# otiliastr/coper

Hardware: NVIDIA B200
Metric: train_rows_per_s (higher is better)
Workload: dtype fp16x3

## Files before the change

### coper_b200/csrc/common.cuh

```cuda
#pragma once
#include <cuda_runtime.h>
#include <stdint.h>
#include "../../include/coper.h"

namespace coper {

extern thread_local int g_last_cuda_error;
extern long long g_launch_count;

inline int check_launch() {
  ++g_launch_count;
  cudaError_t e = cudaPeekAtLastError();
  if (e != cudaSuccess) {
    g_last_cuda_error = (int)e;
    cudaGetLastError();
    return COPER_ERR_CUDA;
  }
  return COPER_OK;
}
inline int check_cuda(cudaError_t e) {
  if (e != cudaSuccess) {
    g_last_cuda_error = (int)e;
    return COPER_ERR_CUDA;
  }
  return COPER_OK;
}
#define COPER_CHECK_ARG(cond) \
  do {                        \
    if (!(cond)) return COPER_ERR_INVALID_ARG; \
  } while (0)

static inline cudaStream_t as_stream(coper_stream_t s) { return reinterpret_cast<cudaStream_t>(s); }

__device__ __forceinline__ void pdl_trigger() { asm volatile("griddepcontrol.launch_dependents;" ::: "memory"); }
__device__ __forceinline__ void pdl_wait() { asm volatile("griddepcontrol.wait;" ::: "memory"); }
__device__ __forceinline__ void pdl_enter() {
  pdl_trigger();
  pdl_wait();
}
bool pdl_enabled();
template <typename... KArgs, typename... Args>
inline void launch_pdl(void (*kernel)(KArgs...), dim3 grid, dim3 block, size_t smem, cudaStream_t st, Args&&... args) {
  cudaLaunchConfig_t cfg = {};
  cfg.gridDim = grid;
  cfg.blockDim = block;
  cfg.dynamicSmemBytes = smem;
  cfg.stream = st;
  cudaLaunchAttribute attr[1];
  attr[0].id = cudaLaunchAttributeProgrammaticStreamSerialization;
  attr[0].val.programmaticStreamSerializationAllowed = pdl_enabled() ? 1 : 0;
  cfg.attrs = attr;
  cfg.numAttrs = 1;
  cudaLaunchKernelEx(&cfg, kernel, static_cast<KArgs>(args)...);
}

__host__ __device__ __forceinline__ uint32_t hash32(uint64_t seed, uint64_t idx) {
  uint64_t z = seed + (idx + 1) * 0x9E3779B97F4A7C15ull;
  z = (z ^ (z >> 30)) * 0xBF58476D1CE4E5B9ull;
  z = (z ^ (z >> 27)) * 0x94D049BB133111EBull;
  z ^= (z >> 31);
  return (uint32_t)(z >> 32);
}
__host__ __device__ __forceinline__ uint32_t keep_threshold(float keep) {
  double t = (double)keep * 4294967296.0;
  if (t >= 4294967295.0) return 0xFFFFFFFFu;
  if (t <= 0.0) return 0u;
  return (uint32_t)t;
}
__device__ __forceinline__ float drop_factor(float keep, float inv_keep, uint32_t thr, uint64_t seed, uint64_t idx) {
  if (keep >= 1.0f) return 1.0f;
  return hash32(seed, idx) < thr ? inv_keep : 0.0f;
}

__device__ __forceinline__ float bn_bwd_dx(float dout, float post_factor, float xv, float ac, float bc, float mean,
                                           float invstd, float c1, float c2, int relu) {
  float g = __fmul_rn(dout, post_factor);
  if (relu && !(fmaf(ac, xv, bc) > 0.f)) g = 0.f;
  const float xhat = __fmul_rn(__fsub_rn(xv, mean), invstd);
  return __fmul_rn(ac, fmaf(-xhat, c2, __fsub_rn(g, c1)));
}

__device__ __forceinline__ float warp_sum(float v) {
#pragma unroll
  for (int o = 16; o > 0; o >>= 1) v += __shfl_xor_sync(0xffffffffu, v, o);
  return v;
}
__device__ __forceinline__ float warp_max(float v) {
#pragma unroll
  for (int o = 16; o > 0; o >>= 1) v = fmaxf(v, __shfl_xor_sync(0xffffffffu, v, o));
  return v;
}
__device__ __forceinline__ double warp_sum_d(double v) {
#pragma unroll
  for (int o = 16; o > 0; o >>= 1) v += __shfl_xor_sync(0xffffffffu, v, o);
  return v;
}
__device__ __forceinline__ int warp_sum_i(int v) {
#pragma unroll
  for (int o = 16; o > 0; o >>= 1) v += __shfl_xor_sync(0xffffffffu, v, o);
  return v;
}

template <typename T>
__device__ __forceinline__ T block_sum(T v, T* smem32) {
  int lane = threadIdx.x & 31, w = threadIdx.x >> 5;
#pragma unroll
  for (int o = 16; o > 0; o >>= 1) v += __shfl_xor_sync(0xffffffffu, v, o);
  if (lane == 0) smem32[w] = v;
  __syncthreads();
  T r = T(0);
  if (w == 0) {
    int nw = (blockDim.x + 31) >> 5;
    r = lane < nw ? smem32[lane] : T(0);
#pragma unroll
    for (int o = 16; o > 0; o >>= 1) r += __shfl_xor_sync(0xffffffffu, r, o);
  }
  __syncthreads();
  return r;
}

constexpr int kFp16x3TargetExp = 10;
__host__ __device__ __forceinline__ int fp16x3_exponent_of(float absmax) {
  if (!(absmax > 0.f) || !(absmax < 3.0e38f)) return 0;
  int ex;
  frexpf(absmax, &ex);
  int e = kFp16x3TargetExp - (ex - 1);
  return e < -100 ? -100 : (e > 100 ? 100 : e);
}

inline int sm_count() {
  static int cached[64] = {};
  int dev = 0;
  if (cudaGetDevice(&dev) != cudaSuccess || dev < 0 || dev >= 64) return 148;
  if (!cached[dev]) {
    int n = 0;
    if (cudaDeviceGetAttribute(&n, cudaDevAttrMultiProcessorCount, dev) != cudaSuccess || n <= 0) n = 148;
    cached[dev] = n;
  }
  return cached[dev];
}

int reduce_partials_and_sum(const float* in, int S, int64_t n, float scale, int accumulate, float* out,
                            const double* dsum_in, int dsum_n, double* dsum_out, cudaStream_t st);

static inline int ceil_div(int64_t a, int64_t b) { return (int)((a + b - 1) / b); }
static inline size_t align_up(size_t x, size_t a) { return (x + a - 1) / a * a; }

}
```

### coper_b200/csrc/umma.cuh

```cuda
#pragma once
#include <cuda.h>
#include <cuda_bf16.h>
#include "common.cuh"

namespace coper {
namespace umma {

__device__ __forceinline__ uint32_t smem_u32(const void* p) { return (uint32_t)__cvta_generic_to_shared(p); }

__device__ __forceinline__ bool elect_one() {
  uint32_t pred;
  asm volatile("{\n\t.reg .pred P;\n\telect.sync _|P, 0xffffffff;\n\tselp.u32 %0, 1, 0, P;\n\t}" : "=r"(pred));
  return pred != 0;
}
__device__ __forceinline__ int warp_idx_uniform() { return __shfl_sync(0xffffffffu, (int)(threadIdx.x >> 5), 0); }

__device__ __forceinline__ void mbar_init(uint64_t* bar, uint32_t count) {
  asm volatile("mbarrier.init.shared::cta.b64 [%0], %1;" ::"r"(smem_u32(bar)), "r"(count));
}
__device__ __forceinline__ void fence_barrier_init() { asm volatile("fence.mbarrier_init.release.cluster;" ::: "memory"); }
__device__ __forceinline__ void fence_proxy_async() { asm volatile("fence.proxy.async.shared::cta;" ::: "memory"); }
__device__ __forceinline__ void mbar_expect_tx(uint64_t* bar, uint32_t bytes) {
  asm volatile("mbarrier.arrive.expect_tx.shared::cta.b64 _, [%0], %1;" ::"r"(smem_u32(bar)), "r"(bytes) : "memory");
}
__device__ __forceinline__ void mbar_arrive(uint64_t* bar) {
  asm volatile("mbarrier.arrive.shared::cta.b64 _, [%0];" ::"r"(smem_u32(bar)) : "memory");
}
__device__ __forceinline__ void mbar_wait(uint64_t* bar, uint32_t parity) {
  uint32_t addr = smem_u32(bar);
  uint32_t done = 0;
  while (!done) {
    asm volatile(
        "{\n\t.reg .pred p;\n\t"
        "mbarrier.try_wait.parity.shared::cta.b64 p, [%1], %2;\n\t"
        "selp.u32 %0, 1, 0, p;\n\t}"
        : "=r"(done)
        : "r"(addr), "r"(parity)
        : "memory");
  }
}

__device__ __forceinline__ void tma_load_2d(void* dst_smem, const CUtensorMap* tmap, uint64_t* bar, int c0, int c1) {
  asm volatile(
      "cp.async.bulk.tensor.2d.shared::cluster.global.mbarrier::complete_tx::bytes [%0], [%1, {%3, %4}], [%2];"
      ::"r"(smem_u32(dst_smem)), "l"(reinterpret_cast<uint64_t>(tmap)), "r"(smem_u32(bar)), "r"(c0), "r"(c1)
      : "memory");
}
__device__ __forceinline__ void tma_store_2d(const CUtensorMap* tmap, const void* src_smem, int c0, int c1) {
  asm volatile("cp.async.bulk.tensor.2d.global.shared::cta.bulk_group [%0, {%2, %3}], [%1];"
               ::"l"(reinterpret_cast<uint64_t>(tmap)), "r"(smem_u32(src_smem)), "r"(c0), "r"(c1)
               : "memory");
}
__device__ __forceinline__ void tma_store_commit() { asm volatile("cp.async.bulk.commit_group;" ::: "memory"); }
__device__ __forceinline__ void tma_store_wait_read() { asm volatile("cp.async.bulk.wait_group.read 0;" ::: "memory"); }
__device__ __forceinline__ void tma_store_wait_all() { asm volatile("cp.async.bulk.wait_group 0;" ::: "memory"); }
__device__ __forceinline__ void mbar_wait_guarded(uint64_t* bar, uint32_t parity) {
  uint32_t addr = smem_u32(bar);
  uint32_t done = 0;
  long long t0 = 0;
  for (uint32_t spins = 0; !done; ++spins) {
    asm volatile(
        "{\n\t.reg .pred p;\n\t"
        "mbarrier.try_wait.parity.shared::cta.b64 p, [%1], %2;\n\t"
        "selp.u32 %0, 1, 0, p;\n\t}"
        : "=r"(done)
        : "r"(addr), "r"(parity)
        : "memory");
    if (!done && (spins & 1023u) == 1023u) {
      long long now = clock64();
      if (t0 == 0) t0 = now;
      else if (now - t0 > 4000000000ll) __trap();
    }
  }
}
__device__ __forceinline__ void tma_prefetch_l2_2d(const CUtensorMap* tmap, int c0, int c1) {
  asm volatile("cp.async.bulk.prefetch.tensor.2d.L2.global.tile [%0, {%1, %2}];"
               ::"l"(reinterpret_cast<uint64_t>(tmap)), "r"(c0), "r"(c1)
               : "memory");
}
__device__ __forceinline__ void tma_prefetch_desc(const CUtensorMap* tmap) {
  asm volatile("prefetch.tensormap [%0];" ::"l"(reinterpret_cast<uint64_t>(tmap)) : "memory");
}

__device__ __forceinline__ void tmem_alloc(uint32_t* smem_dst, uint32_t ncols) {
  asm volatile("tcgen05.alloc.cta_group::1.sync.aligned.shared::cta.b32 [%0], %1;" ::"r"(smem_u32(smem_dst)), "r"(ncols)
               : "memory");
}
__device__ __forceinline__ void tmem_relinquish() {
  asm volatile("tcgen05.relinquish_alloc_permit.cta_group::1.sync.aligned;" ::: "memory");
}
__device__ __forceinline__ void tmem_dealloc(uint32_t taddr, uint32_t ncols) {
  asm volatile("tcgen05.dealloc.cta_group::1.sync.aligned.b32 %0, %1;" ::"r"(taddr), "r"(ncols) : "memory");
}
__device__ __forceinline__ void tc_fence_before() { asm volatile("tcgen05.fence::before_thread_sync;" ::: "memory"); }
__device__ __forceinline__ void tc_fence_after() { asm volatile("tcgen05.fence::after_thread_sync;" ::: "memory"); }

__device__ __forceinline__ void mma_bf16(uint32_t tmem_d, uint64_t desc_a, uint64_t desc_b, uint32_t idesc, uint32_t acc) {
  asm volatile(
      "{\n\t.reg .pred p;\n\tsetp.ne.b32 p, %4, 0;\n\t"
      "tcgen05.mma.cta_group::1.kind::f16 [%0], %1, %2, %3, p;\n\t}"
      ::"r"(tmem_d), "l"(desc_a), "l"(desc_b), "r"(idesc), "r"(acc)
      : "memory");
}
__device__ __forceinline__ void mma_tf32(uint32_t tmem_d, uint64_t desc_a, uint64_t desc_b, uint32_t idesc, uint32_t acc) {
  asm volatile(
      "{\n\t.reg .pred p;\n\tsetp.ne.b32 p, %4, 0;\n\t"
      "tcgen05.mma.cta_group::1.kind::tf32 [%0], %1, %2, %3, p;\n\t}"
      ::"r"(tmem_d), "l"(desc_a), "l"(desc_b), "r"(idesc), "r"(acc)
      : "memory");
}
__device__ __forceinline__ void mma_commit(uint64_t* bar) {
  asm volatile("tcgen05.commit.cta_group::1.mbarrier::arrive::one.shared::cluster.b64 [%0];" ::"r"(smem_u32(bar))
               : "memory");
}

__device__ __forceinline__ void tmem_ld32(uint32_t taddr, uint32_t (&r)[32]) {
  asm volatile(
      "tcgen05.ld.sync.aligned.32x32b.x32.b32 "
      "{%0, %1, %2, %3, %4, %5, %6, %7, %8, %9, %10, %11, %12, %13, %14, %15, "
      "%16, %17, %18, %19, %20, %21, %22, %23, %24, %25, %26, %27, %28, %29, %30, %31}, [%32];"
      : "=r"(r[0]), "=r"(r[1]), "=r"(r[2]), "=r"(r[3]), "=r"(r[4]), "=r"(r[5]), "=r"(r[6]), "=r"(r[7]), "=r"(r[8]),
        "=r"(r[9]), "=r"(r[10]), "=r"(r[11]), "=r"(r[12]), "=r"(r[13]), "=r"(r[14]), "=r"(r[15]), "=r"(r[16]),
        "=r"(r[17]), "=r"(r[18]), "=r"(r[19]), "=r"(r[20]), "=r"(r[21]), "=r"(r[22]), "=r"(r[23]), "=r"(r[24]),
        "=r"(r[25]), "=r"(r[26]), "=r"(r[27]), "=r"(r[28]), "=r"(r[29]), "=r"(r[30]), "=r"(r[31])
      : "r"(taddr)
      : "memory");
}
__device__ __forceinline__ void tmem_ld16(uint32_t taddr, uint32_t (&r)[16]) {
  asm volatile(
      "tcgen05.ld.sync.aligned.32x32b.x16.b32 "
      "{%0, %1, %2, %3, %4, %5, %6, %7, %8, %9, %10, %11, %12, %13, %14, %15}, [%16];"
      : "=r"(r[0]), "=r"(r[1]), "=r"(r[2]), "=r"(r[3]), "=r"(r[4]), "=r"(r[5]), "=r"(r[6]), "=r"(r[7]), "=r"(r[8]),
        "=r"(r[9]), "=r"(r[10]), "=r"(r[11]), "=r"(r[12]), "=r"(r[13]), "=r"(r[14]), "=r"(r[15])
      : "r"(taddr)
      : "memory");
}
__device__ __forceinline__ void tmem_ld_wait() { asm volatile("tcgen05.wait::ld.sync.aligned;" ::: "memory"); }

enum : uint32_t { LAYOUT_SW128 = 2, LAYOUT_SW128_BASE32B = 1 };
__device__ __forceinline__ uint64_t make_desc(uint32_t smem_addr, uint32_t lbo_bytes, uint32_t sbo_bytes,
                                              uint32_t layout_type = LAYOUT_SW128) {
  uint64_t d = 0;
  d |= (uint64_t)((smem_addr & 0x3FFFFu) >> 4);
  d |= (uint64_t)((lbo_bytes >> 4) & 0x3FFFu) << 16;
  d |= (uint64_t)((sbo_bytes >> 4) & 0x3FFFu) << 32;
  d |= (uint64_t)1 << 46;
  d |= (uint64_t)layout_type << 61;
  return d;
}
__device__ __forceinline__ uint64_t make_desc_kmajor(uint32_t smem_addr) { return make_desc(smem_addr, 16, 1024); }

enum : uint32_t { FMT_F16 = 0, FMT_BF16 = 1, FMT_TF32 = 2 };
__host__ __device__ constexpr uint32_t make_idesc(uint32_t fmt, uint32_t M, uint32_t N, uint32_t a_mn, uint32_t b_mn) {
  return (1u << 4) | (fmt << 7) | (fmt << 10) | (a_mn << 15) | (b_mn << 16) | ((N >> 3) << 17) | ((M >> 4) << 24);
}

typedef CUresult (*EncodeTiledFn)(CUtensorMap*, CUtensorMapDataType, cuuint32_t, void*, const cuuint64_t*,
                                  const cuuint64_t*, const cuuint32_t*, const cuuint32_t*, CUtensorMapInterleave,
                                  CUtensorMapSwizzle, CUtensorMapL2promotion, CUtensorMapFloatOOBfill);
EncodeTiledFn get_encode_fn();

int make_tmap_2d(CUtensorMap* out, const void* base, int elem_bytes, bool is_bf16, uint64_t rows, uint64_t cols,
                 uint64_t pitch_elems, uint32_t box_cols, uint32_t box_rows, bool atom32 = false);

}
}
```

### coper_b200/csrc/umma_cpg.cu

```cuda
#include <cuda_fp16.h>
#include "umma_gemm.cuh"

namespace coper {
using namespace umma;

size_t tc_prepared_bytes(int64_t rows, int cols, int prec);
int tc_prepare(const float* src, int64_t rows, int cols, int64_t ld_src, int prec, void* dst, cudaStream_t st);
int64_t tc_prepared_ld(int cols, int prec);
TcOperand tc_operand(const void* prep, int64_t rows, int cols, int prec);
void* tc_fp16x3_trailer(const void* prep, int64_t rows, int cols);
int tc_gemm_store(int prec, bool a_mn, bool b_mn, const TcOperand& A, const TcOperand& B, const GemmProblem& p,
                  bool split, const StoreEpi& epi, cudaStream_t st);

struct CpgFwdEpi : EpiBase {
  static constexpr bool kAccumulate = true;
  const float* c;
  int dc;
  float* out;
  long long ld, split_stride;
  __device__ __forceinline__ float group_scale(const GemmProblem& p, const TileCoord& t, int row) const {
    return row < p.M ? __ldg(c + (long long)row * dc + t.group) : 0.f;
  }
  __device__ __forceinline__ void chunk(const GemmProblem& p, const TileCoord& t, int row, int col,
                                        const uint32_t (&r)[32], int) const {
    if (row >= p.M) return;
    float* o = out + t.split * split_stride + (long long)row * ld + col;
    if (col + 31 < p.N && ((reinterpret_cast<uintptr_t>(o) & 15) == 0)) {
#pragma unroll
      for (int j = 0; j < 32; j += 4)
        *reinterpret_cast<float4*>(o + j) = make_float4(__uint_as_float(r[j]), __uint_as_float(r[j + 1]),
                                                        __uint_as_float(r[j + 2]), __uint_as_float(r[j + 3]));
    } else {
#pragma unroll
      for (int j = 0; j < 32; ++j)
        if (col + j < p.N) o[j] = __uint_as_float(r[j]);
    }
  }
};

template <int PREC>
using CpgFwdCfg = GemmCfg<PREC, 256, (PREC == PREC_BF16 ? 4 : 2), 8, false, true,
                          (PREC == PREC_BF16 ? 0 : PREC == PREC_FP16X3 ? 2 : 4)>;

struct CpgFwdPlan {
  GemmProblem p;
  size_t off_f, off_P, off_slabs, total;
};
static CpgFwdPlan cpg_fwd_plan(int B, int dc, int F, int d, int prec) {
  CpgFwdPlan L;
  GemmProblem p{};
  p.M = B; p.N = d; p.K = F; p.groups = dc; p.groups_inner = 1;
  p.a_group_mn = 0; p.a_group_k = 0; p.b_group_mn = 0; p.b_group_k = F;
  if (prec == COPER_PREC_BF16) plan_gemm<CpgFwdCfg<PREC_BF16>>(p, true);
  else if (prec == COPER_PREC_FP16X3) plan_gemm<CpgFwdCfg<PREC_FP16X3>>(p, true);
  else plan_gemm<CpgFwdCfg<PREC_TF32X3>>(p, true);
  L.p = p;
  size_t o = 0;
  L.off_f = o; o = align_up(o + tc_prepared_bytes(B, F, prec), 256);
  L.off_P = o; o = align_up(o + tc_prepared_bytes((int64_t)dc * F, d, prec), 256);
  L.off_slabs = o; o = align_up(o + (size_t)p.splits * B * d * sizeof(float), 256);
  L.total = o;
  return L;
}

struct CpgBwdTEpi : EpiBase {
  static constexpr bool kAccumulate = true;
  const float* c;
  const float* f;
  int dc;
  float* df;
  float* dc_part;
  float freg[32];
  float fsum;
  __device__ __forceinline__ void tile_begin(const GemmProblem& p, const TileCoord&, int row, int col0) {
    fsum = 0.f;
    if (row < p.M && col0 < p.N) {
      const float4* src = reinterpret_cast<const float4*>(f + (long long)row * p.N + col0);
#pragma unroll
      for (int j = 0; j < 8; ++j) {
        float4 v = __ldg(src + j);
        freg[4 * j] = v.x; freg[4 * j + 1] = v.y; freg[4 * j + 2] = v.z; freg[4 * j + 3] = v.w;
      }
    } else {
#pragma unroll
      for (int j = 0; j < 32; ++j) freg[j] = 0.f;
    }
  }
  __device__ __forceinline__ float group_scale(const GemmProblem& p, const TileCoord& t, int row) const {
    return row < p.M ? __ldg(c + (long long)row * dc + t.group) : 0.f;
  }
  __device__ __forceinline__ void group_vals(const GemmProblem&, const TileCoord&, int, int, const uint32_t (&v)[16],
                                             int half_idx) {
#pragma unroll
    for (int j = 0; j < 16; ++j) fsum = fmaf(freg[(half_idx & 1) * 16 + j], __uint_as_float(v[j]), fsum);
  }
  __device__ __forceinline__ void group_done(const GemmProblem& p, const TileCoord& t, int row, int col_group,
                                             int col_groups) {
    if (row < p.M)
      dc_part[((long long)(t.n_blk * col_groups + col_group) * p.M + row) * dc + t.group] = fsum;
    fsum = 0.f;
  }
  __device__ __forceinline__ void chunk(const GemmProblem& p, const TileCoord&, int row, int col,
                                        const uint32_t (&r)[32], int) const {
    if (row >= p.M) return;
    float4* o = reinterpret_cast<float4*>(df + (long long)row * p.N + col);
#pragma unroll
    for (int j = 0; j < 8; ++j)
      o[j] = make_float4(__uint_as_float(r[4 * j]), __uint_as_float(r[4 * j + 1]), __uint_as_float(r[4 * j + 2]),
                         __uint_as_float(r[4 * j + 3]));
  }
};
constexpr int kBwdTEpiWarps = 16;
constexpr int kBwdTBlockN = 128;
template <int PREC>
using CpgBwdTCfg = GemmCfg<PREC, kBwdTBlockN, (PREC == PREC_BF16 ? 4 : 3), kBwdTEpiWarps, false, false, 0>;

__global__ void absmax_scaled_kernel(const float* __restrict__ dy, const float* __restrict__ c, int B, int d, int dc,
                                     uint32_t* __restrict__ trailer) {
  pdl_enter();
  const int lane = threadIdx.x & 31;
  for (int b = blockIdx.x * (blockDim.x >> 5) + (threadIdx.x >> 5); b < B; b += gridDim.x * (blockDim.x >> 5)) {
    float my = 0.f, mc = 0.f;
    for (int j = lane; j < d; j += 32) my = fmaxf(my, fabsf(__ldg(dy + (int64_t)b * d + j)));
    for (int g = lane; g < dc; g += 32) mc = fmaxf(mc, fabsf(__ldg(c + (int64_t)b * dc + g)));
#pragma unroll
    for (int o = 16; o > 0; o >>= 1) {
      my = fmaxf(my, __shfl_xor_sync(0xffffffffu, my, o));
      mc = fmaxf(mc, __shfl_xor_sync(0xffffffffu, mc, o));
    }
    const float m = my * mc;
    if (lane == 0 && m > 0.f) atomicMax(trailer + 1, __float_as_uint(m));
  }
}
__global__ void prepare_scaled_kernel(const float* __restrict__ dy, const float* __restrict__ c, int B, int d, int dc,
                                      int64_t ldp, int prec, void* __restrict__ dst, uint32_t* __restrict__ trailer) {
  pdl_enter();
  int64_t n = (int64_t)dc * B * ldp;
  int64_t stride = (int64_t)gridDim.x * blockDim.x;
  float sc = 1.0f;
  if (prec == COPER_PREC_FP16X3) {
    const int ex = fp16x3_exponent_of(__uint_as_float(trailer[1]));
    if (blockIdx.x == 0 && threadIdx.x == 0) reinterpret_cast<int*>(trailer)[0] = ex;
    sc = exp2f((float)ex);
  }
  for (int64_t e = (int64_t)blockIdx.x * blockDim.x + threadIdx.x; e < n; e += stride) {
    int64_t r = e / ldp;
    int j = (int)(e - r * ldp);
    int g = (int)(r / B), b = (int)(r - (int64_t)g * B);
    float x = j < d ? __ldg(dy + (int64_t)b * d + j) * __ldg(c + (int64_t)b * dc + g) : 0.f;
    if (prec == COPER_PREC_BF16) {
      static_cast<__nv_bfloat16*>(dst)[e] = __float2bfloat16_rn(x);
    } else if (prec == COPER_PREC_FP16X3) {
      const float xs = x * sc;
      const __half h = __float2half_rn(xs);
      static_cast<__half*>(dst)[e] = h;
      static_cast<__half*>(dst)[n + e] = __float2half_rn(xs - __half2float(h));
    } else {
      uint32_t h;
      asm("cvt.rna.tf32.f32 %0, %1;" : "=r"(h) : "f"(x));
      float hf = __uint_as_float(h);
      static_cast<float*>(dst)[e] = hf;
      static_cast<float*>(dst)[n + e] = x - hf;
    }
  }
}

__global__ void __launch_bounds__(256) cpg_bwd_prepare_fp16x3_kernel(const float* __restrict__ dy,
                                                                     const float* __restrict__ c, int B, int d, int dc,
                                                                     int64_t ldp, __half* __restrict__ dyp,
                                                                     __half* __restrict__ dycp,
                                                                     uint32_t* __restrict__ tr_dy,
                                                                     uint32_t* __restrict__ tr_dyc) {
  pdl_enter();
  __shared__ float wmax[2][8];
  const int lane = threadIdx.x & 31, warp = threadIdx.x >> 5;
  float m_dy = 0.f, m_dyc = 0.f;
  for (int b = blockIdx.x * 8 + warp; b < B; b += gridDim.x * 8) {
    float my = 0.f, mc = 0.f;
    for (int j = lane; j < d; j += 32) my = fmaxf(my, fabsf(__ldg(dy + (int64_t)b * d + j)));
    for (int g = lane; g < dc; g += 32) mc = fmaxf(mc, fabsf(__ldg(c + (int64_t)b * dc + g)));
    my = warp_max(my);
    mc = warp_max(mc);
    m_dy = fmaxf(m_dy, my);
    m_dyc = fmaxf(m_dyc, my * mc);
  }
  if (lane == 0) { wmax[0][warp] = m_dy; wmax[1][warp] = m_dyc; }
  __syncthreads();
  if (threadIdx.x == 0) {
#pragma unroll
    for (int w = 1; w < 8; ++w) { m_dy = fmaxf(m_dy, wmax[0][w]); m_dyc = fmaxf(m_dyc, wmax[1][w]); }
    if (m_dy > 0.f) atomicMax(tr_dy + 1, __float_as_uint(m_dy));
    if (m_dyc > 0.f) atomicMax(tr_dy + 4, __float_as_uint(m_dyc));
    __threadfence();
    atomicAdd(tr_dy + 3, 1u);
    const long long t0 = clock64();
    while (*reinterpret_cast<volatile uint32_t*>(tr_dy + 3) < gridDim.x) {
      if (clock64() - t0 > 4000000000ll) __trap();
    }
    __threadfence();
  }
  __syncthreads();
  const uint32_t bits_dy = *reinterpret_cast<volatile uint32_t*>(tr_dy + 1);
  const uint32_t bits_dyc = *reinterpret_cast<volatile uint32_t*>(tr_dy + 4);
  const int e_dy = fp16x3_exponent_of(__uint_as_float(bits_dy)), e_dyc = fp16x3_exponent_of(__uint_as_float(bits_dyc));
  if (blockIdx.x == 0 && threadIdx.x == 0) {
    reinterpret_cast<int*>(tr_dy)[0] = e_dy;
    tr_dy[2] = bits_dy;
    reinterpret_cast<int*>(tr_dyc)[0] = e_dyc;
    tr_dyc[1] = bits_dyc;
  }
  const float sc_dy = exp2f((float)e_dy), sc_dyc = exp2f((float)e_dyc);
  const int gpr = (int)(ldp / 8);
  const int64_t per = (int64_t)B * gpr, units = per * (1 + dc);
  __half* const dy_lo = dyp + (int64_t)B * ldp;
  __half* const dyc_lo = dycp + (int64_t)dc * B * ldp;
  for (int64_t u = (int64_t)blockIdx.x * 256 + threadIdx.x; u < units; u += (int64_t)gridDim.x * 256) {
    const int p = (int)(u / per);
    const int64_t v = u - (int64_t)p * per;
    const int b = (int)(v / gpr), c0 = (int)(v - (int64_t)b * gpr) * 8;
    const float cs = p == 0 ? 1.0f : __ldg(c + (int64_t)b * dc + (p - 1));
    const float sc = p == 0 ? sc_dy : sc_dyc;
    __half2 h[4], l[4];
#pragma unroll
    for (int k = 0; k < 4; ++k) {
      const int j = c0 + 2 * k;
      float x0 = j < d ? __ldg(dy + (int64_t)b * d + j) : 0.f, x1 = j + 1 < d ? __ldg(dy + (int64_t)b * d + j + 1) : 0.f;
      if (p != 0) { x0 = j < d ? x0 * cs : 0.f; x1 = j + 1 < d ? x1 * cs : 0.f; }
      const float a0 = x0 * sc, a1 = x1 * sc;
      h[k] = __floats2half2_rn(a0, a1);
      const float2 hf = __half22float2(h[k]);
      l[k] = __floats2half2_rn(a0 - hf.x, a1 - hf.y);
    }
    __half* hi = p == 0 ? dyp + v * 8 : dycp + ((int64_t)(p - 1) * per + v) * 8;
    __half* lo = p == 0 ? dy_lo + v * 8 : dyc_lo + ((int64_t)(p - 1) * per + v) * 8;
    *reinterpret_cast<uint4*>(hi) = *reinterpret_cast<uint4*>(h);
    *reinterpret_cast<uint4*>(lo) = *reinterpret_cast<uint4*>(l);
  }
}

struct CpgBwdPlan {
  size_t off_f, off_P, off_dy, off_dyc, off_dcpart, total;
  int dc_slabs;
};
static CpgBwdPlan cpg_bwd_plan(int B, int dc, int F, int d, int prec) {
  CpgBwdPlan L;
  size_t o = 0;
  L.off_f = o; o = align_up(o + tc_prepared_bytes(B, F, prec), 256);
  L.off_P = o; o = align_up(o + tc_prepared_bytes((int64_t)dc * F, d, prec), 256);
  L.off_dy = o; o = align_up(o + tc_prepared_bytes(B, d, prec), 256);
  L.off_dyc = o; o = align_up(o + tc_prepared_bytes((int64_t)dc * B, d, prec), 256);
  L.dc_slabs = ((F + kBwdTBlockN - 1) / kBwdTBlockN) * (kBwdTEpiWarps / 4);
  L.off_dcpart = o; o = align_up(o + (size_t)L.dc_slabs * B * dc * sizeof(float), 256);
  L.total = o;
  return L;
}

size_t umma_cpg_fwd_workspace_bytes(int B, int dc, int F, int d, int prec) { return cpg_fwd_plan(B, dc, F, d, prec).total; }
size_t umma_cpg_bwd_workspace_bytes(int B, int dc, int F, int d, int prec) {
  size_t a = cpg_bwd_plan(B, dc, F, d, prec).total, b = cpg_fwd_plan(B, dc, F, d, prec).total;
  return a > b ? a : b;
}

int umma_cpg_fwd_partials(const float* c, const float* f, const float* P, const void* P_prepared, int B, int dc, int F,
                          int d, void* ws, size_t ws_bytes, int prec, cudaStream_t st, float** slabs, int* n_slabs) {
  if (F % 32 != 0 || d > 256) return COPER_ERR_UNSUPPORTED;
  CpgFwdPlan L = cpg_fwd_plan(B, dc, F, d, prec);
  if (!ws || ws_bytes < L.total) return COPER_ERR_WORKSPACE;
  if (reinterpret_cast<uintptr_t>(ws) & 255) return COPER_ERR_INVALID_ARG;
  char* w = static_cast<char*>(ws);
  void* fp = w + L.off_f;
  const void* Pp = P_prepared ? P_prepared : w + L.off_P;
  float* out = reinterpret_cast<float*>(w + L.off_slabs);
  int rc;
  if ((rc = tc_prepare(f, B, F, F, prec, fp, st))) return rc;
  if (!P_prepared && (rc = tc_prepare(P, (int64_t)dc * F, d, d, prec, w + L.off_P, st))) return rc;
  CpgFwdEpi epi;
  epi.c = c; epi.dc = dc; epi.out = out; epi.ld = d; epi.split_stride = (long long)B * d;
  TcOperand A = tc_operand(fp, B, F, prec), Bo = tc_operand(Pp, (int64_t)dc * F, d, prec);
  if (prec == COPER_PREC_BF16) rc = launch_gemm<CpgFwdCfg<PREC_BF16>, CpgFwdEpi>(A, Bo, L.p, epi, st);
  else if (prec == COPER_PREC_FP16X3) rc = launch_gemm<CpgFwdCfg<PREC_FP16X3>, CpgFwdEpi>(A, Bo, L.p, epi, st);
  else rc = launch_gemm<CpgFwdCfg<PREC_TF32X3>, CpgFwdEpi>(A, Bo, L.p, epi, st);
  *slabs = out;
  *n_slabs = L.p.splits;
  return rc;
}

int umma_cpg_bwd(const float* c, const float* f, const float* P, const void* P_prepared, const float* dy, int B, int dc,
                 int F, int d, float* dP, float* df, float* dc_out, void* ws, size_t ws_bytes, int prec,
                 int flags, cudaStream_t st) {
  if (F % 32 != 0 || d > 256) return COPER_ERR_UNSUPPORTED;
  const bool inputs = !(flags & COPER_CPG_BWD_WEIGHT_GRADS_ONLY), weights = !(flags & COPER_CPG_BWD_INPUT_GRADS_ONLY);
  CpgBwdPlan L = cpg_bwd_plan(B, dc, F, d, prec);
  if (!ws || ws_bytes < L.total) return COPER_ERR_WORKSPACE;
  if (reinterpret_cast<uintptr_t>(ws) & 255) return COPER_ERR_INVALID_ARG;
  char* w = static_cast<char*>(ws);
  void* fp = w + L.off_f;
  const void* Pp = P_prepared ? P_prepared : w + L.off_P;
  void* dyp = w + L.off_dy;
  void* dycp = w + L.off_dyc;
  float* dc_part = reinterpret_cast<float*>(w + L.off_dcpart);
  int rc = COPER_OK;
  if (inputs) {
    if (!(flags & COPER_CPG_BWD_REUSE_FWD)) {
      if ((rc = tc_prepare(f, B, F, F, prec, fp, st))) return rc;
      if (!P_prepared && (rc = tc_prepare(P, (int64_t)dc * F, d, d, prec, w + L.off_P, st))) return rc;
    }
    int64_t ldp = tc_prepared_ld(d, prec);
    int64_t n = (int64_t)dc * B * ldp;
    if (prec == COPER_PREC_FP16X3 && n <= ((int64_t)8 << 20)) {
      uint32_t* tr_dy = static_cast<uint32_t*>(tc_fp16x3_trailer(dyp, B, d));
      uint32_t* tr_dyc = static_cast<uint32_t*>(tc_fp16x3_trailer(dycp, (int64_t)dc * B, d));
      if ((rc = check_cuda(cudaMemsetAsync(tr_dy, 0, 32, st)))) return rc;
      const int64_t want = ((int64_t)(1 + dc) * B * (ldp / 8) + 256 * 4 - 1) / (256 * 4);
      int g = (int)(want < (int64_t)sm_count() * 2 ? want : (int64_t)sm_count() * 2);
      if (g < 1) g = 1;
      launch_pdl(cpg_bwd_prepare_fp16x3_kernel, g, 256, 0, st, dy, c, B, d, dc, ldp, static_cast<__half*>(dyp),
                 static_cast<__half*>(dycp), tr_dy, tr_dyc);
      if ((rc = check_launch())) return rc;
    } else {
      if ((rc = tc_prepare(dy, B, d, d, prec, dyp, st))) return rc;
      int grid = (int)((n + 255) / 256 < sm_count() * 8 ? (n + 255) / 256 : sm_count() * 8);
      uint32_t* trailer = nullptr;
      if (prec == COPER_PREC_FP16X3) {
        trailer = static_cast<uint32_t*>(tc_fp16x3_trailer(dycp, (int64_t)dc * B, d));
        if ((rc = check_cuda(cudaMemsetAsync(trailer, 0, 8, st)))) return rc;
        launch_pdl(absmax_scaled_kernel, (B + 7) / 8, 256, 0, st, dy, c, B, d, dc, trailer);
        if ((rc = check_launch())) return rc;
      }
      launch_pdl(prepare_scaled_kernel, grid, 256, 0, st, dy, c, B, d, dc, ldp, prec, dycp, trailer);
      if ((rc = check_launch())) return rc;
    }
    GemmProblem p{};
    p.M = B; p.N = F; p.K = d; p.groups = dc; p.groups_inner = 1;
    p.a_group_mn = 0; p.a_group_k = 0; p.b_group_mn = F; p.b_group_k = 0;
    CpgBwdTEpi epi;
    epi.c = c; epi.f = f; epi.dc = dc; epi.df = df; epi.dc_part = dc_part; epi.fsum = 0.f;
    TcOperand A = tc_operand(dyp, B, d, prec), Bo = tc_operand(Pp, (int64_t)dc * F, d, prec);
    if (prec == COPER_PREC_BF16) {
      plan_gemm<CpgBwdTCfg<PREC_BF16>>(p, false);
      rc = launch_gemm<CpgBwdTCfg<PREC_BF16>, CpgBwdTEpi>(A, Bo, p, epi, st);
    } else if (prec == COPER_PREC_FP16X3) {
      plan_gemm<CpgBwdTCfg<PREC_FP16X3>>(p, false);
      rc = launch_gemm<CpgBwdTCfg<PREC_FP16X3>, CpgBwdTEpi>(A, Bo, p, epi, st);
    } else {
      plan_gemm<CpgBwdTCfg<PREC_TF32X3>>(p, false);
      rc = launch_gemm<CpgBwdTCfg<PREC_TF32X3>, CpgBwdTEpi>(A, Bo, p, epi, st);
    }
    if (rc) return rc;
    if ((rc = coper_reduce_partials(dc_part, L.dc_slabs, (int64_t)B * dc, 1.0f, 0, dc_out, (coper_stream_t)st)))
      return rc;
  }
  if (weights) {
    GemmProblem p{};
    p.M = F; p.N = d; p.K = B; p.groups = dc; p.groups_inner = 0;
    p.a_group_mn = 0; p.a_group_k = 0; p.b_group_mn = 0; p.b_group_k = B;
    StoreEpi epi = make_store_epi(dP, d, (long long)F * d, 0);
    rc = tc_gemm_store(prec, true, true, tc_operand(fp, B, F, prec), tc_operand(dycp, (int64_t)dc * B, d, prec), p,
                       false, epi, st);
  }
  return rc;
}

}
```

### coper_b200/csrc/umma_gemm.cu

```cuda
#include "umma_gemm.cuh"

namespace coper {
using namespace umma;

size_t tc_prepared_bytes(int64_t rows, int cols, int prec);
int tc_prepare(const float* src, int64_t rows, int cols, int64_t ld_src, int prec, void* dst, cudaStream_t st);
int64_t tc_prepared_ld(int cols, int prec);
void* tc_fp16x3_trailer(const void* prep, int64_t rows, int cols);

template <int PREC, bool A_MN, bool B_MN>
using StoreCfg = GemmCfg<PREC, 256, (PREC == PREC_BF16 ? 4 : 2), (PREC == PREC_BF16 ? 4 : 8), A_MN, B_MN,
                         (PREC == PREC_BF16 ? 0 : PREC == PREC_FP16X3 ? 2 : 4)>;

template <int PREC>
static int dispatch_layout(bool a_mn, bool b_mn, const TcOperand& A, const TcOperand& B, GemmProblem p, bool split,
                           const StoreEpi& epi, cudaStream_t st) {
  if (!a_mn && !b_mn) { plan_gemm<StoreCfg<PREC, false, false>>(p, split); return launch_gemm<StoreCfg<PREC, false, false>>(A, B, p, epi, st); }
  if (!a_mn && b_mn)  { plan_gemm<StoreCfg<PREC, false, true>>(p, split);  return launch_gemm<StoreCfg<PREC, false, true>>(A, B, p, epi, st); }
  if (a_mn && !b_mn)  { plan_gemm<StoreCfg<PREC, true, false>>(p, split);  return launch_gemm<StoreCfg<PREC, true, false>>(A, B, p, epi, st); }
  plan_gemm<StoreCfg<PREC, true, true>>(p, split);
  return launch_gemm<StoreCfg<PREC, true, true>>(A, B, p, epi, st);
}

using ResBCfg = GemmCfg<PREC_BF16, 128, 4, 8, false, true, 0, 8>;
int tc_gemm_store_resident_b(const TcOperand& A, const TcOperand& B, GemmProblem p, const StoreEpi& epi, cudaStream_t st) {
  plan_gemm<ResBCfg>(p, false);
  return launch_gemm<ResBCfg>(A, B, p, epi, st);
}
bool tc_resident_b_ok(int prec, bool a_mn, bool b_mn, const GemmProblem& p) {
  return prec == COPER_PREC_BF16 && !a_mn && b_mn && p.groups == 1 && p.K <= ResBCfg::RES_KB * ResBCfg::BLOCK_K &&
         p.M >= 16 * BLOCK_M;
}

int tc_gemm_store(int prec, bool a_mn, bool b_mn, const TcOperand& A, const TcOperand& B, const GemmProblem& p,
                  bool split, const StoreEpi& epi, cudaStream_t st) {
  if (prec == COPER_PREC_BF16) return dispatch_layout<PREC_BF16>(a_mn, b_mn, A, B, p, split, epi, st);
  if (prec == COPER_PREC_TF32X3) return dispatch_layout<PREC_TF32X3>(a_mn, b_mn, A, B, p, split, epi, st);
  if (prec == COPER_PREC_FP16X3) return dispatch_layout<PREC_FP16X3>(a_mn, b_mn, A, B, p, split, epi, st);
  return COPER_ERR_UNSUPPORTED;
}
int tc_plan_splits(int prec, GemmProblem p, bool split) {
  if (prec == COPER_PREC_BF16) plan_gemm<StoreCfg<PREC_BF16, false, false>>(p, split);
  else if (prec == COPER_PREC_FP16X3) plan_gemm<StoreCfg<PREC_FP16X3, false, false>>(p, split);
  else plan_gemm<StoreCfg<PREC_TF32X3, false, false>>(p, split);
  return p.splits;
}

TcOperand tc_operand(const void* prep, int64_t rows, int cols, int prec) {
  TcOperand o;
  int64_t ldp = tc_prepared_ld(cols, prec);
  o.main = prep;
  o.lo = prec == COPER_PREC_TF32X3 ? static_cast<const void*>(static_cast<const float*>(prep) + rows * ldp)
         : prec == COPER_PREC_FP16X3 ? static_cast<const void*>(static_cast<const uint16_t*>(prep) + rows * ldp)
                                     : nullptr;
  o.exp = prec == COPER_PREC_FP16X3 ? static_cast<const int*>(tc_fp16x3_trailer(prep, rows, cols)) : nullptr;
  o.rows = (uint64_t)rows;
  o.cols = (uint64_t)cols;
  o.pitch = (uint64_t)ldp;
  return o;
}
}

using namespace coper;

extern "C" {

size_t coper_tc_gemm_workspace_bytes(int M, int N, int K, int prec) {
  size_t a = tc_prepared_bytes(M > K ? M : K, M > K ? K : M, prec) + tc_prepared_bytes(K, M, prec);
  size_t b = tc_prepared_bytes(N > K ? N : K, N > K ? K : N, prec) + tc_prepared_bytes(K, N, prec);
  return a + b + 1024;
}

int coper_tc_gemm(int transA, int transB, int M, int N, int K, const float* A, int lda, const float* B, int ldb,
                  float* C, int ldc, int prec, void* workspace, size_t workspace_bytes, coper_stream_t stream) {
  COPER_CHECK_ARG(A && B && C && workspace && M > 0 && N > 0 && K > 0 && ldc >= N);
  if (prec != COPER_PREC_BF16 && prec != COPER_PREC_TF32X3 && prec != COPER_PREC_FP16X3) return COPER_ERR_UNSUPPORTED;
  if (workspace_bytes < coper_tc_gemm_workspace_bytes(M, N, K, prec)) return COPER_ERR_WORKSPACE;
  cudaStream_t st = as_stream(stream);
  char* p = reinterpret_cast<char*>((reinterpret_cast<uintptr_t>(workspace) + 255) & ~uintptr_t(255));
  int64_t a_rows = transA ? K : M, a_cols = transA ? M : K;
  int64_t b_rows = transB ? N : K, b_cols = transB ? K : N;
  void* Ap = p;
  void* Bp = p + tc_prepared_bytes(a_rows, (int)a_cols, prec);
  int rc;
  if ((rc = tc_prepare(A, a_rows, (int)a_cols, lda, prec, Ap, st))) return rc;
  if ((rc = tc_prepare(B, b_rows, (int)b_cols, ldb, prec, Bp, st))) return rc;
  GemmProblem g{};
  g.M = M; g.N = N; g.K = K; g.groups = 1; g.groups_inner = 0;
  StoreEpi epi = make_store_epi(C, ldc, 0, 0);
  return tc_gemm_store(prec, transA != 0, transB == 0, tc_operand(Ap, a_rows, (int)a_cols, prec),
                       tc_operand(Bp, b_rows, (int)b_cols, prec), g, false, epi, st);
}

}
```

### coper_b200/csrc/umma_gemm.cuh

```cuda
#pragma once
#include "umma.cuh"

namespace coper {
namespace umma {

constexpr int PREC_BF16 = COPER_PREC_BF16, PREC_TF32X3 = COPER_PREC_TF32X3, PREC_FP16X3 = COPER_PREC_FP16X3;
constexpr int BLOCK_M = 128;
constexpr int NUM_NON_EPI_THREADS = 128;

template <int PREC_, int BLOCK_N_, int STAGES_, int EPI_WARPS_, bool A_MN_, bool B_MN_, int PROMOTE_KB_ = 0,
          int RES_KB_ = 0>
struct GemmCfg {
  static constexpr int PROMOTE_KB = PROMOTE_KB_;
  static constexpr int RES_KB = RES_KB_;
  static constexpr int PREC = PREC_, BLOCK_N = BLOCK_N_, STAGES = STAGES_, EPI_WARPS = EPI_WARPS_;
  static constexpr bool A_MN = A_MN_, B_MN = B_MN_;
  static constexpr int ELEM = (PREC == PREC_TF32X3) ? 4 : 2;
  static constexpr int CHUNK = 128 / ELEM;
  static constexpr int BLOCK_K = CHUNK;
  static constexpr int UMMA_K = 32 / ELEM;
  static constexpr int TERMS = (PREC == PREC_BF16) ? 1 : 2;
  static constexpr bool SCALED = (PREC == PREC_FP16X3);
  static constexpr int A_BYTES = BLOCK_M * 128;
  static constexpr int B_BYTES = BLOCK_N * 128;
  static constexpr int STAGE_BYTES = RES_KB_ > 0 ? TERMS * A_BYTES : TERMS * (A_BYTES + B_BYTES);
  static constexpr int RES_BYTES = RES_KB_ * TERMS * B_BYTES;
  static constexpr int TMEM_COLS = (2 * BLOCK_N <= 32) ? 32 : (2 * BLOCK_N <= 64) ? 64 : (2 * BLOCK_N <= 128) ? 128
                                   : (2 * BLOCK_N <= 256) ? 256 : 512;
  static constexpr int THREADS = NUM_NON_EPI_THREADS + EPI_WARPS * 32;
  static constexpr size_t SMEM_BYTES = (size_t)STAGES * STAGE_BYTES + RES_BYTES + 1024  + 256 ;

  static constexpr uint32_t FMT = (PREC == PREC_BF16) ? FMT_BF16 : (PREC == PREC_FP16X3) ? FMT_F16 : FMT_TF32;
  static constexpr bool MN_ATOM32 = (PREC == PREC_TF32X3);
  static constexpr uint32_t MN_LAYOUT = MN_ATOM32 ? LAYOUT_SW128_BASE32B : LAYOUT_SW128;
  static constexpr uint32_t MN_SBO = MN_ATOM32 ? 512 : 1024;
  static constexpr uint32_t IDESC = make_idesc(FMT, BLOCK_M, BLOCK_N, A_MN ? 1u : 0u, B_MN ? 1u : 0u);
  static_assert(BLOCK_N % 16 == 0 && BLOCK_N >= 16 && BLOCK_N <= 256, "UMMA N");
  static_assert(2 * BLOCK_N <= 512, "TMEM double buffer");
  static_assert(!A_MN || (BLOCK_M % CHUNK == 0), "MN-major A chunking");
  static_assert(!B_MN || (BLOCK_N % CHUNK == 0), "MN-major B chunking");
};

template <class Cfg>
struct SmemLayout {
  uint8_t* base;
  uint64_t* full;
  uint64_t* empty;
  uint64_t* tfull;
  uint64_t* tempty;
  uint64_t* bfull;
  uint32_t* tmem_ptr;
  uint8_t* res;
  __device__ __forceinline__ explicit SmemLayout(uint8_t* raw) {
    base = reinterpret_cast<uint8_t*>((reinterpret_cast<uintptr_t>(raw) + 1023) & ~uintptr_t(1023));
    res = base + (size_t)Cfg::STAGES * Cfg::STAGE_BYTES;
    uint64_t* bars = reinterpret_cast<uint64_t*>(res + Cfg::RES_BYTES);
    full = bars;
    empty = bars + Cfg::STAGES;
    tfull = bars + 2 * Cfg::STAGES;
    tempty = tfull + 2;
    bfull = tempty + 2;
    tmem_ptr = reinterpret_cast<uint32_t*>(bfull + 1);
  }
  __device__ __forceinline__ uint8_t* res_plane(int kb, int term) const {
    return res + ((size_t)kb * Cfg::TERMS + term) * Cfg::B_BYTES;
  }
  __device__ __forceinline__ uint8_t* a_plane(int stage, int term) const {
    return base + (size_t)stage * Cfg::STAGE_BYTES + term * Cfg::A_BYTES;
  }
  __device__ __forceinline__ uint8_t* b_plane(int stage, int term) const {
    return base + (size_t)stage * Cfg::STAGE_BYTES + Cfg::TERMS * Cfg::A_BYTES + term * Cfg::B_BYTES;
  }
};

template <class Cfg>
__device__ __forceinline__ uint32_t cta_setup(const SmemLayout<Cfg>& sm) {
  int warp = threadIdx.x >> 5;
  if (warp == 1 && (threadIdx.x & 31) == 0) {
    for (int i = 0; i < Cfg::STAGES; ++i) { mbar_init(&sm.full[i], 1); mbar_init(&sm.empty[i], 1); }
    for (int i = 0; i < 2; ++i) { mbar_init(&sm.tfull[i], 1); mbar_init(&sm.tempty[i], Cfg::EPI_WARPS); }
    mbar_init(sm.bfull, 1);
    fence_barrier_init();
  } else if (warp == 2) {
    tmem_alloc(sm.tmem_ptr, Cfg::TMEM_COLS);
    tmem_relinquish();
  }
  tc_fence_before();
  __syncthreads();
  tc_fence_after();
  return *sm.tmem_ptr;
}
template <class Cfg>
__device__ __forceinline__ void cta_teardown(uint32_t tmem_base) {
  tc_fence_before();
  __syncthreads();
  if ((threadIdx.x >> 5) == 2) {
    tc_fence_after();
    tmem_dealloc(tmem_base, Cfg::TMEM_COLS);
  }
}

template <class Cfg>
__device__ __forceinline__ void produce_stage(const SmemLayout<Cfg>& sm, int stage, const CUtensorMap* tA,
                                              const CUtensorMap* tAlo, const CUtensorMap* tB, const CUtensorMap* tBlo,
                                              int a_mn0, int b_mn0, int a_k0, int b_k0, bool leader) {
  uint64_t* bar = &sm.full[stage];
  if (leader) mbar_expect_tx(bar, Cfg::STAGE_BYTES);
#pragma unroll
  for (int t = 0; t < Cfg::TERMS; ++t) {
    const CUtensorMap* ma = t ? tAlo : tA;
    const CUtensorMap* mb = t ? tBlo : tB;
    if (!Cfg::A_MN) {
      if (leader) tma_load_2d(sm.a_plane(stage, t), ma, bar, a_k0, a_mn0);
    } else {
#pragma unroll
      for (int c = 0; c < BLOCK_M / Cfg::CHUNK; ++c)
        if (leader) tma_load_2d(sm.a_plane(stage, t) + c * (Cfg::BLOCK_K * 128), ma, bar, a_mn0 + c * Cfg::CHUNK, a_k0);
    }
    if (Cfg::RES_KB > 0) {
    } else if (!Cfg::B_MN) {
      if (leader) tma_load_2d(sm.b_plane(stage, t), mb, bar, b_k0, b_mn0);
    } else {
#pragma unroll
      for (int c = 0; c < Cfg::BLOCK_N / Cfg::CHUNK; ++c)
        if (leader) tma_load_2d(sm.b_plane(stage, t) + c * (Cfg::BLOCK_K * 128), mb, bar, b_mn0 + c * Cfg::CHUNK, b_k0);
    }
  }
}

template <class Cfg>
__device__ __forceinline__ void issue_stage_rt(const SmemLayout<Cfg>& sm, int stage, uint32_t tmem_d, int kvalid,
                                               bool first, uint32_t idesc, int kb_res, bool leader) {
  const int nk = (kvalid + Cfg::UMMA_K - 1) / Cfg::UMMA_K;
  uint64_t da[2], db[2];
#pragma unroll
  for (int t = 0; t < Cfg::TERMS; ++t) {
    const uint32_t a_addr = smem_u32(sm.a_plane(stage, t));
    const uint32_t b_addr = smem_u32(Cfg::RES_KB > 0 ? sm.res_plane(kb_res, t) : sm.b_plane(stage, t));
    da[t] = Cfg::A_MN ? make_desc(a_addr, Cfg::BLOCK_K * 128, Cfg::MN_SBO, Cfg::MN_LAYOUT) : make_desc_kmajor(a_addr);
    db[t] = Cfg::B_MN ? make_desc(b_addr, Cfg::BLOCK_K * 128, Cfg::MN_SBO, Cfg::MN_LAYOUT) : make_desc_kmajor(b_addr);
  }
  constexpr uint64_t a_step = (Cfg::A_MN ? Cfg::UMMA_K * 128 : 32) >> 4, b_step = (Cfg::B_MN ? Cfg::UMMA_K * 128 : 32) >> 4;
  constexpr int NK_MAX = Cfg::BLOCK_K / Cfg::UMMA_K;
  if (leader) {
#pragma unroll
    for (int k = 0; k < NK_MAX; ++k) {
      if (k < nk) {
        const uint32_t acc = (first && k == 0) ? 0u : 1u;
        if (Cfg::PREC == PREC_BF16) {
          mma_bf16(tmem_d, da[0] + k * a_step, db[0] + k * b_step, idesc, acc);
        } else if (Cfg::PREC == PREC_FP16X3) {
          mma_bf16(tmem_d, da[1] + k * a_step, db[0] + k * b_step, idesc, acc);
          mma_bf16(tmem_d, da[0] + k * a_step, db[1] + k * b_step, idesc, 1u);
          mma_bf16(tmem_d, da[0] + k * a_step, db[0] + k * b_step, idesc, 1u);
        } else {
          mma_tf32(tmem_d, da[1] + k * a_step, db[0] + k * b_step, idesc, acc);
          mma_tf32(tmem_d, da[0] + k * a_step, db[1] + k * b_step, idesc, 1u);
          mma_tf32(tmem_d, da[0] + k * a_step, db[0] + k * b_step, idesc, 1u);
        }
      }
    }
  }
  __syncwarp();
}

struct PipeState {
  int stage = 0;
  uint32_t phase = 0;
  template <int STAGES>
  __device__ __forceinline__ void advance() {
    if (++stage == STAGES) { stage = 0; phase ^= 1; }
  }
};

}
}

namespace coper {
namespace umma {

struct GemmProblem {
  int M, N, K;
  int m_tiles, n_tiles;
  int splits, kb_per_split;
  int groups;
  int groups_inner;
  int a_group_mn, a_group_k;
  int b_group_mn, b_group_k;
  const int* exp_a;
  const int* exp_b;
  float post_scale;
  int n_fastest;
};
struct TileCoord {
  int group, split, m_blk, n_blk, kb0, kb1;
};

struct EpiBase {
  static constexpr bool kAccumulate = false;
  __device__ __forceinline__ void tile_begin(const GemmProblem&, const TileCoord&, int, int) {}
  __device__ __forceinline__ void tile_prefetch(const GemmProblem&, const TileCoord&, int, int) {}
  __device__ __forceinline__ float group_scale(const GemmProblem&, const TileCoord&, int) const { return 1.0f; }
  __device__ __forceinline__ void group_vals(const GemmProblem&, const TileCoord&, int, int, const uint32_t (&)[16],
                                             int) {}
  __device__ __forceinline__ void group_done(const GemmProblem&, const TileCoord&, int, int, int) {}
  __device__ __forceinline__ void tile_done(const GemmProblem&, const TileCoord&, int, int, int) {}
  __device__ __forceinline__ void finish(int, int) {}
};

__device__ __forceinline__ long long gemm_supers(const GemmProblem& p) {
  return (long long)p.m_tiles * p.n_tiles * p.splits * (p.groups_inner ? 1 : p.groups);
}
__device__ __forceinline__ TileCoord gemm_decode(const GemmProblem& p, long long s, int g_inner, int block_k) {
  TileCoord t;
  if (p.n_fastest) {
    t.n_blk = (int)(s % p.n_tiles); s /= p.n_tiles;
    t.m_blk = (int)(s % p.m_tiles); s /= p.m_tiles;
  } else {
    t.m_blk = (int)(s % p.m_tiles); s /= p.m_tiles;
    t.n_blk = (int)(s % p.n_tiles); s /= p.n_tiles;
  }
  t.split = (int)(s % p.splits);  s /= p.splits;
  t.group = p.groups_inner ? g_inner : (int)s;
  int kb_total = (p.K + block_k - 1) / block_k;
  t.kb0 = t.split * p.kb_per_split;
  t.kb1 = min(kb_total, t.kb0 + p.kb_per_split);
  return t;
}

template <class Cfg, class Epi>
__global__ void __launch_bounds__(Cfg::THREADS, 1)
umma_gemm_kernel(const __grid_constant__ CUtensorMap tA, const __grid_constant__ CUtensorMap tAlo,
                 const __grid_constant__ CUtensorMap tB, const __grid_constant__ CUtensorMap tBlo,
                 const GemmProblem p, Epi epi) {
  coper::pdl_trigger();
  extern __shared__ uint8_t smem_raw[];
  SmemLayout<Cfg> sm(smem_raw);
  uint32_t tmem_base = cta_setup<Cfg>(sm);
  coper::pdl_wait();
  const int warp = warp_idx_uniform(), lane = threadIdx.x & 31;
  const long long supers = gemm_supers(p);
  const int g_loop = p.groups_inner ? p.groups : 1;

  if (warp == 0) {
    const bool leader = elect_one();
    if (leader) {
      tma_prefetch_desc(&tA);
      tma_prefetch_desc(&tB);
    }
    PipeState ps;
    int res_nblk = -1;
    for (long long s = blockIdx.x; s < supers; s += gridDim.x) {
      for (int g = 0; g < g_loop; ++g) {
        TileCoord t = gemm_decode(p, s, g, Cfg::BLOCK_K);
        int a_mn0 = t.m_blk * BLOCK_M + t.group * p.a_group_mn;
        int b_mn0 = t.n_blk * Cfg::BLOCK_N + t.group * p.b_group_mn;
        if (Cfg::RES_KB > 0 && t.n_blk != res_nblk) {
          PipeState q = ps;
          for (int i = 0; i < Cfg::STAGES; ++i) {
            mbar_wait(&sm.empty[q.stage], q.phase ^ 1);
            q.template advance<Cfg::STAGES>();
          }
          const int kbn = t.kb1 - t.kb0;
          if (leader) mbar_expect_tx(sm.bfull, (uint32_t)(kbn * Cfg::TERMS * Cfg::B_BYTES));
          for (int kb = t.kb0; kb < t.kb1; ++kb)
#pragma unroll
            for (int tm = 0; tm < Cfg::TERMS; ++tm) {
              if (!Cfg::B_MN) {
                if (leader)
                  tma_load_2d(sm.res_plane(kb - t.kb0, tm), tm ? &tBlo : &tB, sm.bfull, kb * Cfg::BLOCK_K, b_mn0);
              } else {
#pragma unroll
                for (int c = 0; c < Cfg::BLOCK_N / Cfg::CHUNK; ++c)
                  if (leader)
                    tma_load_2d(sm.res_plane(kb - t.kb0, tm) + c * (Cfg::BLOCK_K * 128), tm ? &tBlo : &tB, sm.bfull,
                                b_mn0 + c * Cfg::CHUNK, kb * Cfg::BLOCK_K);
              }
            }
          res_nblk = t.n_blk;
        }
        for (int kb = t.kb0; kb < t.kb1; ++kb) {
          mbar_wait(&sm.empty[ps.stage], ps.phase ^ 1);
          produce_stage<Cfg>(sm, ps.stage, &tA, &tAlo, &tB, &tBlo, a_mn0, b_mn0,
                             kb * Cfg::BLOCK_K + t.group * p.a_group_k, kb * Cfg::BLOCK_K + t.group * p.b_group_k, leader);
          ps.template advance<Cfg::STAGES>();
        }
      }
    }
    __syncwarp();
  } else if (warp == 1) {
    const bool leader = elect_one();
    PipeState ps;
    int as = 0;
    uint32_t aphase = 0;
    int res_nblk = -1;
    uint32_t bphase = 0;
    for (long long s = blockIdx.x; s < supers; s += gridDim.x) {
      for (int g = 0; g < g_loop; ++g) {
        TileCoord t = gemm_decode(p, s, g, Cfg::BLOCK_K);
        if (Cfg::RES_KB > 0 && t.n_blk != res_nblk) {
          mbar_wait(sm.bfull, bphase);
          bphase ^= 1;
          res_nblk = t.n_blk;
        }
        int n_rem = p.N - t.n_blk * Cfg::BLOCK_N;
        int n_eff = min(Cfg::BLOCK_N, (n_rem + 15) & ~15);
        uint32_t idesc = make_idesc(Cfg::FMT, BLOCK_M, (uint32_t)n_eff, Cfg::A_MN ? 1u : 0u, Cfg::B_MN ? 1u : 0u);
        const int chain = Cfg::PROMOTE_KB > 0 ? Cfg::PROMOTE_KB : (t.kb1 - t.kb0);
        for (int kc = t.kb0; kc < t.kb1; kc += chain) {
          int kce = min(t.kb1, kc + chain);
          mbar_wait(&sm.tempty[as], aphase ^ 1);
          tc_fence_after();
          for (int kb = kc; kb < kce; ++kb) {
            mbar_wait(&sm.full[ps.stage], ps.phase);
            tc_fence_after();
            int kvalid = min(Cfg::BLOCK_K, p.K - kb * Cfg::BLOCK_K);
            issue_stage_rt<Cfg>(sm, ps.stage, tmem_base + as * Cfg::BLOCK_N, kvalid, kb == kc, idesc, kb - t.kb0, leader);
            if (leader) mma_commit(&sm.empty[ps.stage]);
            ps.template advance<Cfg::STAGES>();
          }
          if (leader) mma_commit(&sm.tfull[as]);
          __syncwarp();
          as ^= 1;
          if (as == 0) aphase ^= 1;
        }
      }
    }
  } else if (warp >= 4) {
    const int quarter = warp & 3;
    const int group_c = (warp - 4) >> 2;
    constexpr int GROUPS = Cfg::EPI_WARPS / 4;
    constexpr int COLS = Cfg::BLOCK_N / GROUPS;
    constexpr int NCH = COLS / 32;
    static_assert(COLS % 32 == 0, "epilogue column split");
    int as = 0;
    uint32_t aphase = 0;
    const uint32_t lane_base = (uint32_t)(quarter * 32) << 16;
    float acc_scale = 1.0f;
    if (Cfg::SCALED) {
      const int e = (p.exp_a ? __ldg(p.exp_a) : 0) + (p.exp_b ? __ldg(p.exp_b) : 0);
      acc_scale = exp2f((float)-e) * (p.post_scale != 0.f ? p.post_scale : 1.0f);
    }
    for (long long s = blockIdx.x; s < supers; s += gridDim.x) {
      TileCoord t = gemm_decode(p, s, 0, Cfg::BLOCK_K);
      const int row = t.m_blk * BLOCK_M + quarter * 32 + lane;
      const int col0 = t.n_blk * Cfg::BLOCK_N + group_c * COLS;
      epi.tile_begin(p, t, row, col0);
      if (s + gridDim.x < supers) {
        const TileCoord t2 = gemm_decode(p, s + gridDim.x, 0, Cfg::BLOCK_K);
        epi.tile_prefetch(p, t2, t2.m_blk * BLOCK_M + quarter * 32 + lane, t2.n_blk * Cfg::BLOCK_N + group_c * COLS);
      }
      if constexpr (Cfg::PROMOTE_KB == 0 && !Epi::kAccumulate) {
        mbar_wait(&sm.tfull[as], aphase);
        tc_fence_after();
#pragma unroll
        for (int i = 0; i < NCH; ++i) {
          const int col = col0 + i * 32;
          if (col < p.N) {
            uint32_t r[32];
            tmem_ld32(tmem_base + as * Cfg::BLOCK_N + group_c * COLS + i * 32 + lane_base, r);
            tmem_ld_wait();
            if (Cfg::SCALED) {
#pragma unroll
              for (int j = 0; j < 32; ++j) r[j] = __float_as_uint(__uint_as_float(r[j]) * acc_scale);
            }
            epi.chunk(p, t, row, col, r, i);
          }
        }
        tc_fence_before();
        __syncwarp();
        if (lane == 0) mbar_arrive(&sm.tempty[as]);
        as ^= 1;
        if (as == 0) aphase ^= 1;
      } else {
        float accr[NCH][32];
#pragma unroll
        for (int i = 0; i < NCH; ++i)
#pragma unroll
          for (int j = 0; j < 32; ++j) accr[i][j] = 0.f;
        for (int g = 0; g < g_loop; ++g) {
          t = gemm_decode(p, s, g, Cfg::BLOCK_K);
          const float scale = epi.group_scale(p, t, row);
          const int chain = Cfg::PROMOTE_KB > 0 ? Cfg::PROMOTE_KB : (t.kb1 - t.kb0);
          for (int kc = t.kb0; kc < t.kb1; kc += chain) {
            mbar_wait(&sm.tfull[as], aphase);
            tc_fence_after();
#pragma unroll
            for (int i = 0; i < NCH; ++i) {
              if (col0 + i * 32 < p.N) {
#pragma unroll
                for (int h = 0; h < 2; ++h) {
                  uint32_t r[16];
                  tmem_ld16(tmem_base + as * Cfg::BLOCK_N + group_c * COLS + i * 32 + h * 16 + lane_base, r);
                  tmem_ld_wait();
                  if (Cfg::SCALED) {
#pragma unroll
                    for (int j = 0; j < 16; ++j) r[j] = __float_as_uint(__uint_as_float(r[j]) * acc_scale);
                  }
                  epi.group_vals(p, t, row, col0 + i * 32 + h * 16, r, i * 2 + h);
#pragma unroll
                  for (int j = 0; j < 16; ++j) accr[i][h * 16 + j] = fmaf(scale, __uint_as_float(r[j]), accr[i][h * 16 + j]);
                }
              }
            }
            tc_fence_before();
            __syncwarp();
            if (lane == 0) mbar_arrive(&sm.tempty[as]);
            as ^= 1;
            if (as == 0) aphase ^= 1;
          }
          epi.group_done(p, t, row, group_c, GROUPS);
        }
#pragma unroll
        for (int i = 0; i < NCH; ++i) {
          const int col = col0 + i * 32;
          if (col < p.N) {
            uint32_t r[32];
#pragma unroll
            for (int j = 0; j < 32; ++j) r[j] = __float_as_uint(accr[i][j]);
            epi.chunk(p, t, row, col, r, i);
          }
        }
      }
      epi.tile_done(p, t, row, group_c, GROUPS);
    }
    epi.finish(threadIdx.x - NUM_NON_EPI_THREADS, Cfg::EPI_WARPS * 32);
  }
  cta_teardown<Cfg>(tmem_base);
}

struct TcOperand {
  const void* main;
  const void* lo;
  const int* exp;
  uint64_t rows, cols;
  uint64_t pitch;
};

template <class Cfg>
int make_gemm_tmaps(const TcOperand& A, const TcOperand& B, CUtensorMap* tA, CUtensorMap* tAlo, CUtensorMap* tB,
                    CUtensorMap* tBlo) {
  constexpr bool bf16 = Cfg::ELEM == 2;
  int rc;
  uint32_t a_box_rows = Cfg::A_MN ? Cfg::BLOCK_K : BLOCK_M;
  uint32_t b_box_rows = Cfg::B_MN ? Cfg::BLOCK_K : Cfg::BLOCK_N;
  const bool a32 = Cfg::A_MN && Cfg::MN_ATOM32, b32 = Cfg::B_MN && Cfg::MN_ATOM32;
  if ((rc = make_tmap_2d(tA, A.main, Cfg::ELEM, bf16, A.rows, A.cols, A.pitch, Cfg::CHUNK, a_box_rows, a32))) return rc;
  if ((rc = make_tmap_2d(tB, B.main, Cfg::ELEM, bf16, B.rows, B.cols, B.pitch, Cfg::CHUNK, b_box_rows, b32))) return rc;
  *tAlo = *tA;
  *tBlo = *tB;
  if (Cfg::TERMS == 2) {
    if (!A.lo || !B.lo) return COPER_ERR_INVALID_ARG;
    if ((rc = make_tmap_2d(tAlo, A.lo, Cfg::ELEM, bf16, A.rows, A.cols, A.pitch, Cfg::CHUNK, a_box_rows, a32))) return rc;
    if ((rc = make_tmap_2d(tBlo, B.lo, Cfg::ELEM, bf16, B.rows, B.cols, B.pitch, Cfg::CHUNK, b_box_rows, b32))) return rc;
  }
  return COPER_OK;
}

template <class Cfg, class Epi>
int launch_gemm(const TcOperand& A, const TcOperand& B, const GemmProblem& p, const Epi& epi, cudaStream_t st,
                int grid_override = 0) {
  if (p.groups_inner && !Epi::kAccumulate) return COPER_ERR_INVALID_ARG;
  if (Cfg::RES_KB > 0 && (p.splits != 1 || p.groups != 1 || (p.K + Cfg::BLOCK_K - 1) / Cfg::BLOCK_K > Cfg::RES_KB))
    return COPER_ERR_UNSUPPORTED;
  CUtensorMap tA, tAlo, tB, tBlo;
  int rc = make_gemm_tmaps<Cfg>(A, B, &tA, &tAlo, &tB, &tBlo);
  if (rc) return rc;
  int dev = 0;
  if ((rc = check_cuda(cudaGetDevice(&dev)))) return rc;
  static bool attr_done[64] = {};
  if (dev < 0 || dev >= 64) return COPER_ERR_UNSUPPORTED;
  if (!attr_done[dev]) {
    rc = check_cuda(cudaFuncSetAttribute(umma_gemm_kernel<Cfg, Epi>, cudaFuncAttributeMaxDynamicSharedMemorySize,
                                         (int)Cfg::SMEM_BYTES));
    if (rc) return rc;
    attr_done[dev] = true;
  }
  GemmProblem pp = p;
  if (Cfg::SCALED) {
    if (!pp.exp_a) pp.exp_a = A.exp;
    if (!pp.exp_b) pp.exp_b = B.exp;
  }
  const int sms = sm_count();
  long long supers = (long long)p.m_tiles * p.n_tiles * p.splits * (p.groups_inner ? 1 : p.groups);
  int grid = (int)(supers < sms ? supers : sms);
  if (grid_override > 0 && grid_override < grid) grid = grid_override;
  if (grid < 1) return COPER_ERR_INVALID_ARG;
  launch_pdl(umma_gemm_kernel<Cfg, Epi>, grid, Cfg::THREADS, Cfg::SMEM_BYTES, st, tA, tAlo, tB, tBlo, pp, epi);
  return check_launch();
}

template <class Cfg>
inline void plan_gemm(GemmProblem& p, bool allow_split, int target_ctas = 0) {
  if (target_ctas <= 0) target_ctas = sm_count();
  p.m_tiles = (p.M + BLOCK_M - 1) / BLOCK_M;
  p.n_tiles = (p.N + Cfg::BLOCK_N - 1) / Cfg::BLOCK_N;
  int kb_total = (p.K + Cfg::BLOCK_K - 1) / Cfg::BLOCK_K;
  long long base = (long long)p.m_tiles * p.n_tiles * (p.groups_inner ? 1 : p.groups);
  int splits = 1;
  if (allow_split && base < target_ctas) {
    splits = (int)((target_ctas + base - 1) / base);
    if (splits > kb_total) splits = kb_total;
  }
  p.kb_per_split = (kb_total + splits - 1) / splits;
  p.splits = (kb_total + p.kb_per_split - 1) / p.kb_per_split;
}

__device__ __forceinline__ void staged_store_f32(float4* st, const float (&v)[32], float* out0, long long ld,
                                                 int rows_valid, int cols_valid) {
  const int lane = threadIdx.x & 31;
#pragma unroll
  for (int g = 0; g < 8; ++g)
    st[lane * 8 + (g ^ (lane & 7))] = make_float4(v[4 * g], v[4 * g + 1], v[4 * g + 2], v[4 * g + 3]);
  __syncwarp();
  const int g = lane & 7;
#pragma unroll
  for (int k = 0; k < 8; ++k) {
    const int rr = 4 * k + (lane >> 3);
    const float4 x = st[rr * 8 + (g ^ (rr & 7))];
    if (rr < rows_valid && 4 * g < cols_valid) *reinterpret_cast<float4*>(out0 + (long long)rr * ld + 4 * g) = x;
  }
  __syncwarp();
}
constexpr int kStageWarps = 8;
__device__ __forceinline__ float4* stage_tile() {
  __shared__ float4 stage_s[kStageWarps][256];
  return stage_s[((threadIdx.x >> 5) - 4) & (kStageWarps - 1)];
}

struct StoreEpi : EpiBase {
  float* out;
  long long ld, group_stride, split_stride;
  const float* row_scale;
  int row_scale_ld;
  const float* col_bias;
  int extra_col;
  float* extra_out;
  double* sumsq_part;
  double ss_acc;
  __device__ __forceinline__ void chunk(const GemmProblem& p, const TileCoord& t, int row, int col,
                                        const uint32_t (&r)[32], int) {
    const int lane = threadIdx.x & 31;
    const int n_out = extra_col >= 0 ? min(p.N, extra_col) : p.N;
    if (sumsq_part && row < p.M) {
      float ss = 0.f;
#pragma unroll
      for (int j = 0; j < 32; ++j) {
        const float v = __uint_as_float(r[j]);
        ss = (col + j < n_out) ? fmaf(v, v, ss) : ss;
      }
      ss_acc += (double)ss;
    }
    float* base = out + t.group * group_stride + t.split * split_stride;
    float* o0 = base + (long long)(row - lane) * ld + col;
    const bool vec = !col_bias && !row_scale && extra_col < 0 && ((ld & 3) == 0) && ((n_out & 3) == 0) &&
                     ((reinterpret_cast<uintptr_t>(o0) & 15) == 0);
    if (vec) {
      float v[32];
#pragma unroll
      for (int j = 0; j < 32; ++j) v[j] = __uint_as_float(r[j]);
      staged_store_f32(stage_tile(), v, o0, ld, p.M - (row - lane), n_out - col);
      return;
    }
    if (row >= p.M) return;
    float sc = row_scale ? __ldg(row_scale + (long long)row * row_scale_ld + t.group) : 1.0f;
    float* o = base + (long long)row * ld + col;
    {
#pragma unroll
      for (int j = 0; j < 32; ++j) {
        int cj = col + j;
        if (cj < n_out) o[j] = __uint_as_float(r[j]) * sc + (col_bias ? __ldg(col_bias + cj) : 0.f);
        else if (cj == extra_col && cj < p.N) extra_out[row] = __uint_as_float(r[j]) * sc;
      }
    }
  }
  __device__ __forceinline__ void finish(int epi_thread, int epi_threads) {
    if (!sumsq_part) return;
    const double t = warp_sum_d(ss_acc);
    if ((epi_thread & 31) == 0) sumsq_part[(long long)blockIdx.x * (epi_threads >> 5) + (epi_thread >> 5)] = t;
  }
};

inline StoreEpi make_store_epi(float* out, long long ld, long long group_stride, long long split_stride) {
  StoreEpi e;
  e.out = out; e.ld = ld; e.group_stride = group_stride; e.split_stride = split_stride;
  e.row_scale = nullptr; e.row_scale_ld = 0; e.col_bias = nullptr; e.extra_col = -1; e.extra_out = nullptr;
  e.sumsq_part = nullptr; e.ss_acc = 0.0;
  return e;
}

}
}
```

Measured before the change: 999,900.

## Use 2-SM paired UMMA (cta_group::2) clusters for forward and store GEMMs

```diff
diff --git a/coper_b200/csrc/common.cuh b/coper_b200/csrc/common.cuh
--- a/coper_b200/csrc/common.cuh
+++ b/coper_b200/csrc/common.cuh
@@ -40,18 +40,25 @@
 }
 bool pdl_enabled();
 template <typename... KArgs, typename... Args>
-inline void launch_pdl(void (*kernel)(KArgs...), dim3 grid, dim3 block, size_t smem, cudaStream_t st, Args&&... args) {
+inline void launch_pdl_cluster(void (*kernel)(KArgs...), int cluster_x, dim3 grid, dim3 block, size_t smem,
+                               cudaStream_t st, Args&&... args) {
   cudaLaunchConfig_t cfg = {};
   cfg.gridDim = grid;
   cfg.blockDim = block;
   cfg.dynamicSmemBytes = smem;
   cfg.stream = st;
-  cudaLaunchAttribute attr[1];
+  cudaLaunchAttribute attr[2];
   attr[0].id = cudaLaunchAttributeProgrammaticStreamSerialization;
   attr[0].val.programmaticStreamSerializationAllowed = pdl_enabled() ? 1 : 0;
+  attr[1].id = cudaLaunchAttributeClusterDimension;
+  attr[1].val.clusterDim.x = (unsigned)cluster_x; attr[1].val.clusterDim.y = 1; attr[1].val.clusterDim.z = 1;
   cfg.attrs = attr;
-  cfg.numAttrs = 1;
+  cfg.numAttrs = cluster_x > 1 ? 2 : 1;
   cudaLaunchKernelEx(&cfg, kernel, static_cast<KArgs>(args)...);
+}
+template <typename... KArgs, typename... Args>
+inline void launch_pdl(void (*kernel)(KArgs...), dim3 grid, dim3 block, size_t smem, cudaStream_t st, Args&&... args) {
+  launch_pdl_cluster(kernel, 1, grid, block, smem, st, static_cast<Args&&>(args)...);
 }
 
 __host__ __device__ __forceinline__ uint32_t hash32(uint64_t seed, uint64_t idx) {
diff --git a/coper_b200/csrc/umma.cuh b/coper_b200/csrc/umma.cuh
--- a/coper_b200/csrc/umma.cuh
+++ b/coper_b200/csrc/umma.cuh
@@ -82,36 +82,110 @@
   asm volatile("prefetch.tensormap [%0];" ::"l"(reinterpret_cast<uint64_t>(tmap)) : "memory");
 }
 
+template <bool PAIR = false>
 __device__ __forceinline__ void tmem_alloc(uint32_t* smem_dst, uint32_t ncols) {
-  asm volatile("tcgen05.alloc.cta_group::1.sync.aligned.shared::cta.b32 [%0], %1;" ::"r"(smem_u32(smem_dst)), "r"(ncols)
-               : "memory");
-}
+  if constexpr (PAIR)
+    asm volatile("tcgen05.alloc.cta_group::2.sync.aligned.shared::cta.b32 [%0], %1;" ::"r"(smem_u32(smem_dst)), "r"(ncols)
+                 : "memory");
+  else
+    asm volatile("tcgen05.alloc.cta_group::1.sync.aligned.shared::cta.b32 [%0], %1;" ::"r"(smem_u32(smem_dst)), "r"(ncols)
+                 : "memory");
+}
+template <bool PAIR = false>
 __device__ __forceinline__ void tmem_relinquish() {
-  asm volatile("tcgen05.relinquish_alloc_permit.cta_group::1.sync.aligned;" ::: "memory");
-}
+  if constexpr (PAIR) asm volatile("tcgen05.relinquish_alloc_permit.cta_group::2.sync.aligned;" ::: "memory");
+  else asm volatile("tcgen05.relinquish_alloc_permit.cta_group::1.sync.aligned;" ::: "memory");
+}
+template <bool PAIR = false>
 __device__ __forceinline__ void tmem_dealloc(uint32_t taddr, uint32_t ncols) {
-  asm volatile("tcgen05.dealloc.cta_group::1.sync.aligned.b32 %0, %1;" ::"r"(taddr), "r"(ncols) : "memory");
+  if constexpr (PAIR) asm volatile("tcgen05.dealloc.cta_group::2.sync.aligned.b32 %0, %1;" ::"r"(taddr), "r"(ncols) : "memory");
+  else asm volatile("tcgen05.dealloc.cta_group::1.sync.aligned.b32 %0, %1;" ::"r"(taddr), "r"(ncols) : "memory");
 }
 __device__ __forceinline__ void tc_fence_before() { asm volatile("tcgen05.fence::before_thread_sync;" ::: "memory"); }
 __device__ __forceinline__ void tc_fence_after() { asm volatile("tcgen05.fence::after_thread_sync;" ::: "memory"); }
 
+template <bool PAIR = false>
 __device__ __forceinline__ void mma_bf16(uint32_t tmem_d, uint64_t desc_a, uint64_t desc_b, uint32_t idesc, uint32_t acc) {
-  asm volatile(
-      "{\n\t.reg .pred p;\n\tsetp.ne.b32 p, %4, 0;\n\t"
-      "tcgen05.mma.cta_group::1.kind::f16 [%0], %1, %2, %3, p;\n\t}"
-      ::"r"(tmem_d), "l"(desc_a), "l"(desc_b), "r"(idesc), "r"(acc)
-      : "memory");
-}
+  if constexpr (PAIR)
+    asm volatile(
+        "{\n\t.reg .pred p;\n\tsetp.ne.b32 p, %4, 0;\n\t"
+        "tcgen05.mma.cta_group::2.kind::f16 [%0], %1, %2, %3, p;\n\t}"
+        ::"r"(tmem_d), "l"(desc_a), "l"(desc_b), "r"(idesc), "r"(acc)
+        : "memory");
+  else
+    asm volatile(
+        "{\n\t.reg .pred p;\n\tsetp.ne.b32 p, %4, 0;\n\t"
+        "tcgen05.mma.cta_group::1.kind::f16 [%0], %1, %2, %3, p;\n\t}"
+        ::"r"(tmem_d), "l"(desc_a), "l"(desc_b), "r"(idesc), "r"(acc)
+        : "memory");
+}
+template <bool PAIR = false>
 __device__ __forceinline__ void mma_tf32(uint32_t tmem_d, uint64_t desc_a, uint64_t desc_b, uint32_t idesc, uint32_t acc) {
-  asm volatile(
-      "{\n\t.reg .pred p;\n\tsetp.ne.b32 p, %4, 0;\n\t"
-      "tcgen05.mma.cta_group::1.kind::tf32 [%0], %1, %2, %3, p;\n\t}"
-      ::"r"(tmem_d), "l"(desc_a), "l"(desc_b), "r"(idesc), "r"(acc)
-      : "memory");
-}
+  if constexpr (PAIR)
+    asm volatile(
+        "{\n\t.reg .pred p;\n\tsetp.ne.b32 p, %4, 0;\n\t"
+        "tcgen05.mma.cta_group::2.kind::tf32 [%0], %1, %2, %3, p;\n\t}"
+        ::"r"(tmem_d), "l"(desc_a), "l"(desc_b), "r"(idesc), "r"(acc)
+        : "memory");
+  else
+    asm volatile(
+        "{\n\t.reg .pred p;\n\tsetp.ne.b32 p, %4, 0;\n\t"
+        "tcgen05.mma.cta_group::1.kind::tf32 [%0], %1, %2, %3, p;\n\t}"
+        ::"r"(tmem_d), "l"(desc_a), "l"(desc_b), "r"(idesc), "r"(acc)
+        : "memory");
+}
+template <bool PAIR = false>
 __device__ __forceinline__ void mma_commit(uint64_t* bar) {
-  asm volatile("tcgen05.commit.cta_group::1.mbarrier::arrive::one.shared::cluster.b64 [%0];" ::"r"(smem_u32(bar))
-               : "memory");
+  if constexpr (PAIR)
+    asm volatile("tcgen05.commit.cta_group::2.mbarrier::arrive::one.shared::cluster.multicast::cluster.b64 [%0], %1;"
+                 ::"r"(smem_u32(bar)), "h"((uint16_t)3)
+                 : "memory");
+  else
+    asm volatile("tcgen05.commit.cta_group::1.mbarrier::arrive::one.shared::cluster.b64 [%0];" ::"r"(smem_u32(bar))
+                 : "memory");
+}
+
+__device__ __forceinline__ uint32_t cluster_ctarank() {
+  uint32_t r;
+  asm("mov.u32 %0, %%cluster_ctarank;" : "=r"(r));
+  return r;
+}
+__device__ __forceinline__ void cluster_sync() {
+  asm volatile("barrier.cluster.arrive.release.aligned;\n\tbarrier.cluster.wait.acquire.aligned;" ::: "memory");
+}
+__device__ __forceinline__ uint32_t cluster_addr(const void* p, uint32_t rank) {
+  uint32_t a;
+  asm volatile("mapa.shared::cluster.u32 %0, %1, %2;" : "=r"(a) : "r"(smem_u32(p)), "r"(rank));
+  return a;
+}
+__device__ __forceinline__ void mbar_arrive_cluster(uint32_t bar_cluster_addr) {
+  asm volatile("mbarrier.arrive.release.cluster.shared::cluster.b64 _, [%0];" ::"r"(bar_cluster_addr) : "memory");
+}
+__device__ __forceinline__ void mbar_wait_cluster(uint64_t* bar, uint32_t parity) {
+  uint32_t addr = smem_u32(bar);
+  uint32_t done = 0;
+  long long t0 = 0;
+  for (uint32_t spins = 0; !done; ++spins) {
+    asm volatile(
+        "{\n\t.reg .pred p;\n\t"
+        "mbarrier.try_wait.parity.acquire.cluster.shared::cta.b64 p, [%1], %2;\n\t"
+        "selp.u32 %0, 1, 0, p;\n\t}"
+        : "=r"(done)
+        : "r"(addr), "r"(parity)
+        : "memory");
+    if (!done && (spins & 1023u) == 1023u) {
+      long long now = clock64();
+      if (t0 == 0) t0 = now;
+      else if (now - t0 > 4000000000ll) __trap();
+    }
+  }
+}
+__device__ __forceinline__ void tma_load_2d_pair(void* dst_smem, const CUtensorMap* tmap, uint32_t bar_cluster_addr,
+                                                 int c0, int c1) {
+  asm volatile(
+      "cp.async.bulk.tensor.2d.cta_group::2.shared::cluster.global.mbarrier::complete_tx::bytes [%0], [%1, {%3, %4}], [%2];"
+      ::"r"(smem_u32(dst_smem)), "l"(reinterpret_cast<uint64_t>(tmap)), "r"(bar_cluster_addr), "r"(c0), "r"(c1)
+      : "memory");
 }
 
 __device__ __forceinline__ void tmem_ld32(uint32_t taddr, uint32_t (&r)[32]) {
diff --git a/coper_b200/csrc/umma_cpg.cu b/coper_b200/csrc/umma_cpg.cu
--- a/coper_b200/csrc/umma_cpg.cu
+++ b/coper_b200/csrc/umma_cpg.cu
@@ -39,8 +39,8 @@
 };
 
 template <int PREC>
-using CpgFwdCfg = GemmCfg<PREC, 256, (PREC == PREC_BF16 ? 4 : 2), 8, false, true,
-                          (PREC == PREC_BF16 ? 0 : PREC == PREC_FP16X3 ? 2 : 4)>;
+using CpgFwdCfg = GemmCfg<PREC, 256, (PREC == PREC_BF16 ? 6 : 3), 8, false, true,
+                          (PREC == PREC_BF16 ? 0 : PREC == PREC_FP16X3 ? 2 : 4), 0, true>;
 
 struct CpgFwdPlan {
   GemmProblem p;
@@ -113,7 +113,7 @@
 constexpr int kBwdTEpiWarps = 16;
 constexpr int kBwdTBlockN = 128;
 template <int PREC>
-using CpgBwdTCfg = GemmCfg<PREC, kBwdTBlockN, (PREC == PREC_BF16 ? 4 : 3), kBwdTEpiWarps, false, false, 0>;
+using CpgBwdTCfg = GemmCfg<PREC, kBwdTBlockN, (PREC == PREC_BF16 ? 8 : 4), kBwdTEpiWarps, false, false, 0, 0, true>;
 
 __global__ void absmax_scaled_kernel(const float* __restrict__ dy, const float* __restrict__ c, int B, int d, int dc,
                                      uint32_t* __restrict__ trailer) {
diff --git a/coper_b200/csrc/umma_gemm.cu b/coper_b200/csrc/umma_gemm.cu
--- a/coper_b200/csrc/umma_gemm.cu
+++ b/coper_b200/csrc/umma_gemm.cu
@@ -9,8 +9,8 @@
 void* tc_fp16x3_trailer(const void* prep, int64_t rows, int cols);
 
 template <int PREC, bool A_MN, bool B_MN>
-using StoreCfg = GemmCfg<PREC, 256, (PREC == PREC_BF16 ? 4 : 2), (PREC == PREC_BF16 ? 4 : 8), A_MN, B_MN,
-                         (PREC == PREC_BF16 ? 0 : PREC == PREC_FP16X3 ? 2 : 4)>;
+using StoreCfg = GemmCfg<PREC, 256, (PREC == PREC_BF16 ? 6 : 3), (PREC == PREC_BF16 ? 4 : 8), A_MN, B_MN,
+                         (PREC == PREC_BF16 ? 0 : PREC == PREC_FP16X3 ? 2 : 4), 0, true>;
 
 template <int PREC>
 static int dispatch_layout(bool a_mn, bool b_mn, const TcOperand& A, const TcOperand& B, GemmProblem p, bool split,
diff --git a/coper_b200/csrc/umma_gemm.cuh b/coper_b200/csrc/umma_gemm.cuh
--- a/coper_b200/csrc/umma_gemm.cuh
+++ b/coper_b200/csrc/umma_gemm.cuh
@@ -9,10 +9,12 @@
 constexpr int NUM_NON_EPI_THREADS = 128;
 
 template <int PREC_, int BLOCK_N_, int STAGES_, int EPI_WARPS_, bool A_MN_, bool B_MN_, int PROMOTE_KB_ = 0,
-          int RES_KB_ = 0>
+          int RES_KB_ = 0, bool PAIR_ = false>
 struct GemmCfg {
   static constexpr int PROMOTE_KB = PROMOTE_KB_;
   static constexpr int RES_KB = RES_KB_;
+  static constexpr bool PAIR = PAIR_;
+  static constexpr int CTAS = PAIR ? 2 : 1;
   static constexpr int PREC = PREC_, BLOCK_N = BLOCK_N_, STAGES = STAGES_, EPI_WARPS = EPI_WARPS_;
   static constexpr bool A_MN = A_MN_, B_MN = B_MN_;
   static constexpr int ELEM = (PREC == PREC_TF32X3) ? 4 : 2;
@@ -22,7 +24,8 @@
   static constexpr int TERMS = (PREC == PREC_BF16) ? 1 : 2;
   static constexpr bool SCALED = (PREC == PREC_FP16X3);
   static constexpr int A_BYTES = BLOCK_M * 128;
-  static constexpr int B_BYTES = BLOCK_N * 128;
+  static constexpr int B_ROWS = BLOCK_N / CTAS;
+  static constexpr int B_BYTES = B_ROWS * 128;
   static constexpr int STAGE_BYTES = RES_KB_ > 0 ? TERMS * A_BYTES : TERMS * (A_BYTES + B_BYTES);
   static constexpr int RES_BYTES = RES_KB_ * TERMS * B_BYTES;
   static constexpr int TMEM_COLS = (2 * BLOCK_N <= 32) ? 32 : (2 * BLOCK_N <= 64) ? 64 : (2 * BLOCK_N <= 128) ? 128
@@ -34,11 +37,12 @@
   static constexpr bool MN_ATOM32 = (PREC == PREC_TF32X3);
   static constexpr uint32_t MN_LAYOUT = MN_ATOM32 ? LAYOUT_SW128_BASE32B : LAYOUT_SW128;
   static constexpr uint32_t MN_SBO = MN_ATOM32 ? 512 : 1024;
-  static constexpr uint32_t IDESC = make_idesc(FMT, BLOCK_M, BLOCK_N, A_MN ? 1u : 0u, B_MN ? 1u : 0u);
+  static constexpr uint32_t UMMA_M = BLOCK_M * CTAS;
   static_assert(BLOCK_N % 16 == 0 && BLOCK_N >= 16 && BLOCK_N <= 256, "UMMA N");
   static_assert(2 * BLOCK_N <= 512, "TMEM double buffer");
   static_assert(!A_MN || (BLOCK_M % CHUNK == 0), "MN-major A chunking");
-  static_assert(!B_MN || (BLOCK_N % CHUNK == 0), "MN-major B chunking");
+  static_assert(!B_MN || (B_ROWS % CHUNK == 0), "MN-major B chunking");
+  static_assert(!PAIR || RES_KB == 0, "2-SM mode streams B");
 };
 
 template <class Cfg>
@@ -78,52 +82,61 @@
   int warp = threadIdx.x >> 5;
   if (warp == 1 && (threadIdx.x & 31) == 0) {
     for (int i = 0; i < Cfg::STAGES; ++i) { mbar_init(&sm.full[i], 1); mbar_init(&sm.empty[i], 1); }
-    for (int i = 0; i < 2; ++i) { mbar_init(&sm.tfull[i], 1); mbar_init(&sm.tempty[i], Cfg::EPI_WARPS); }
+    for (int i = 0; i < 2; ++i) { mbar_init(&sm.tfull[i], 1); mbar_init(&sm.tempty[i], Cfg::EPI_WARPS * Cfg::CTAS); }
     mbar_init(sm.bfull, 1);
     fence_barrier_init();
   } else if (warp == 2) {
-    tmem_alloc(sm.tmem_ptr, Cfg::TMEM_COLS);
-    tmem_relinquish();
+    tmem_alloc<Cfg::PAIR>(sm.tmem_ptr, Cfg::TMEM_COLS);
+    tmem_relinquish<Cfg::PAIR>();
   }
   tc_fence_before();
-  __syncthreads();
+  if constexpr (Cfg::PAIR) cluster_sync();
+  else __syncthreads();
   tc_fence_after();
   return *sm.tmem_ptr;
 }
 template <class Cfg>
 __device__ __forceinline__ void cta_teardown(uint32_t tmem_base) {
   tc_fence_before();
-  __syncthreads();
+  if constexpr (Cfg::PAIR) cluster_sync();
+  else __syncthreads();
   if ((threadIdx.x >> 5) == 2) {
     tc_fence_after();
-    tmem_dealloc(tmem_base, Cfg::TMEM_COLS);
-  }
-}
-
+    tmem_dealloc<Cfg::PAIR>(tmem_base, Cfg::TMEM_COLS);
+  }
+}
+
+template <class Cfg>
+__device__ __forceinline__ void tma_load_stage(void* dst, const CUtensorMap* m, const SmemLayout<Cfg>& sm, int stage,
+                                               int c0, int c1) {
+  if constexpr (Cfg::PAIR) tma_load_2d_pair(dst, m, cluster_addr(&sm.full[stage], 0), c0, c1);
+  else tma_load_2d(dst, m, &sm.full[stage], c0, c1);
+}
 template <class Cfg>
 __device__ __forceinline__ void produce_stage(const SmemLayout<Cfg>& sm, int stage, const CUtensorMap* tA,
                                               const CUtensorMap* tAlo, const CUtensorMap* tB, const CUtensorMap* tBlo,
                                               int a_mn0, int b_mn0, int a_k0, int b_k0, bool leader) {
-  uint64_t* bar = &sm.full[stage];
-  if (leader) mbar_expect_tx(bar, Cfg::STAGE_BYTES);
+  if (leader && (!Cfg::PAIR || cluster_ctarank() == 0)) mbar_expect_tx(&sm.full[stage], Cfg::CTAS * Cfg::STAGE_BYTES);
 #pragma unroll
   for (int t = 0; t < Cfg::TERMS; ++t) {
     const CUtensorMap* ma = t ? tAlo : tA;
     const CUtensorMap* mb = t ? tBlo : tB;
     if (!Cfg::A_MN) {
-      if (leader) tma_load_2d(sm.a_plane(stage, t), ma, bar, a_k0, a_mn0);
+      if (leader) tma_load_stage<Cfg>(sm.a_plane(stage, t), ma, sm, stage, a_k0, a_mn0);
     } else {
 #pragma unroll
       for (int c = 0; c < BLOCK_M / Cfg::CHUNK; ++c)
-        if (leader) tma_load_2d(sm.a_plane(stage, t) + c * (Cfg::BLOCK_K * 128), ma, bar, a_mn0 + c * Cfg::CHUNK, a_k0);
+        if (leader)
+          tma_load_stage<Cfg>(sm.a_plane(stage, t) + c * (Cfg::BLOCK_K * 128), ma, sm, stage, a_mn0 + c * Cfg::CHUNK, a_k0);
     }
     if (Cfg::RES_KB > 0) {
     } else if (!Cfg::B_MN) {
-      if (leader) tma_load_2d(sm.b_plane(stage, t), mb, bar, b_k0, b_mn0);
+      if (leader) tma_load_stage<Cfg>(sm.b_plane(stage, t), mb, sm, stage, b_k0, b_mn0);
     } else {
 #pragma unroll
-      for (int c = 0; c < Cfg::BLOCK_N / Cfg::CHUNK; ++c)
-        if (leader) tma_load_2d(sm.b_plane(stage, t) + c * (Cfg::BLOCK_K * 128), mb, bar, b_mn0 + c * Cfg::CHUNK, b_k0);
+      for (int c = 0; c < Cfg::B_ROWS / Cfg::CHUNK; ++c)
+        if (leader)
+          tma_load_stage<Cfg>(sm.b_plane(stage, t) + c * (Cfg::BLOCK_K * 128), mb, sm, stage, b_mn0 + c * Cfg::CHUNK, b_k0);
     }
   }
 }
@@ -147,21 +160,33 @@
     for (int k = 0; k < NK_MAX; ++k) {
       if (k < nk) {
         const uint32_t acc = (first && k == 0) ? 0u : 1u;
+        constexpr bool P2 = Cfg::PAIR;
         if (Cfg::PREC == PREC_BF16) {
-          mma_bf16(tmem_d, da[0] + k * a_step, db[0] + k * b_step, idesc, acc);
+          mma_bf16<P2>(tmem_d, da[0] + k * a_step, db[0] + k * b_step, idesc, acc);
         } else if (Cfg::PREC == PREC_FP16X3) {
-          mma_bf16(tmem_d, da[1] + k * a_step, db[0] + k * b_step, idesc, acc);
-          mma_bf16(tmem_d, da[0] + k * a_step, db[1] + k * b_step, idesc, 1u);
-          mma_bf16(tmem_d, da[0] + k * a_step, db[0] + k * b_step, idesc, 1u);
+          mma_bf16<P2>(tmem_d, da[1] + k * a_step, db[0] + k * b_step, idesc, acc);
+          mma_bf16<P2>(tmem_d, da[0] + k * a_step, db[1] + k * b_step, idesc, 1u);
+          mma_bf16<P2>(tmem_d, da[0] + k * a_step, db[0] + k * b_step, idesc, 1u);
         } else {
-          mma_tf32(tmem_d, da[1] + k * a_step, db[0] + k * b_step, idesc, acc);
-          mma_tf32(tmem_d, da[0] + k * a_step, db[1] + k * b_step, idesc, 1u);
-          mma_tf32(tmem_d, da[0] + k * a_step, db[0] + k * b_step, idesc, 1u);
+          mma_tf32<P2>(tmem_d, da[1] + k * a_step, db[0] + k * b_step, idesc, acc);
+          mma_tf32<P2>(tmem_d, da[0] + k * a_step, db[1] + k * b_step, idesc, 1u);
+          mma_tf32<P2>(tmem_d, da[0] + k * a_step, db[0] + k * b_step, idesc, 1u);
         }
       }
     }
   }
   __syncwarp();
+}
+
+template <class Cfg>
+__device__ __forceinline__ void pipe_wait(uint64_t* bar, uint32_t parity) {
+  if constexpr (Cfg::PAIR) mbar_wait_cluster(bar, parity);
+  else mbar_wait(bar, parity);
+}
+template <class Cfg>
+__device__ __forceinline__ void tmem_release(uint64_t* tempty) {
+  if constexpr (Cfg::PAIR) mbar_arrive_cluster(cluster_addr(tempty, 0));
+  else mbar_arrive(tempty);
 }
 
 struct PipeState {
@@ -208,18 +233,24 @@
   __device__ __forceinline__ void finish(int, int) {}
 };
 
-__device__ __forceinline__ long long gemm_supers(const GemmProblem& p) {
-  return (long long)p.m_tiles * p.n_tiles * p.splits * (p.groups_inner ? 1 : p.groups);
-}
-__device__ __forceinline__ TileCoord gemm_decode(const GemmProblem& p, long long s, int g_inner, int block_k) {
+__host__ __device__ __forceinline__ int gemm_m_items(const GemmProblem& p, int ctas) {
+  return (p.m_tiles + ctas - 1) / ctas;
+}
+__host__ __device__ __forceinline__ long long gemm_supers(const GemmProblem& p, int ctas = 1) {
+  return (long long)gemm_m_items(p, ctas) * p.n_tiles * p.splits * (p.groups_inner ? 1 : p.groups);
+}
+__device__ __forceinline__ TileCoord gemm_decode(const GemmProblem& p, long long s, int g_inner, int block_k,
+                                                 int ctas = 1, int rank = 0) {
   TileCoord t;
+  const int mt = gemm_m_items(p, ctas);
   if (p.n_fastest) {
     t.n_blk = (int)(s % p.n_tiles); s /= p.n_tiles;
-    t.m_blk = (int)(s % p.m_tiles); s /= p.m_tiles;
+    t.m_blk = (int)(s % mt); s /= mt;
   } else {
-    t.m_blk = (int)(s % p.m_tiles); s /= p.m_tiles;
+    t.m_blk = (int)(s % mt); s /= mt;
     t.n_blk = (int)(s % p.n_tiles); s /= p.n_tiles;
   }
+  t.m_blk = t.m_blk * ctas + rank;
   t.split = (int)(s % p.splits);  s /= p.splits;
   t.group = p.groups_inner ? g_inner : (int)s;
   int kb_total = (p.K + block_k - 1) / block_k;
@@ -239,7 +270,9 @@
   uint32_t tmem_base = cta_setup<Cfg>(sm);
   coper::pdl_wait();
   const int warp = warp_idx_uniform(), lane = threadIdx.x & 31;
-  const long long supers = gemm_supers(p);
+  constexpr int CTAS = Cfg::CTAS;
+  const int rank = Cfg::PAIR ? (int)cluster_ctarank() : 0;
+  const long long supers = gemm_supers(p, CTAS);
   const int g_loop = p.groups_inner ? p.groups : 1;
 
   if (warp == 0) {
@@ -250,11 +283,15 @@
     }
     PipeState ps;
     int res_nblk = -1;
-    for (long long s = blockIdx.x; s < supers; s += gridDim.x) {
+    for (long long s = blockIdx.x / CTAS; s < supers; s += gridDim.x / CTAS) {
       for (int g = 0; g < g_loop; ++g) {
-        TileCoord t = gemm_decode(p, s, g, Cfg::BLOCK_K);
+        TileCoord t = gemm_decode(p, s, g, Cfg::BLOCK_K, CTAS, rank);
         int a_mn0 = t.m_blk * BLOCK_M + t.group * p.a_group_mn;
         int b_mn0 = t.n_blk * Cfg::BLOCK_N + t.group * p.b_group_mn;
+        if (Cfg::PAIR && rank == 1) {
+          const int n_eff = min(Cfg::BLOCK_N, (p.N - t.n_blk * Cfg::BLOCK_N + 15) & ~15);
+          b_mn0 += n_eff / 2;
+        }
         if (Cfg::RES_KB > 0 && t.n_blk != res_nblk) {
           PipeState q = ps;
           for (int i = 0; i < Cfg::STAGES; ++i) {
@@ -280,7 +317,7 @@
           res_nblk = t.n_blk;
         }
         for (int kb = t.kb0; kb < t.kb1; ++kb) {
-          mbar_wait(&sm.empty[ps.stage], ps.phase ^ 1);
+          pipe_wait<Cfg>(&sm.empty[ps.stage], ps.phase ^ 1);
           produce_stage<Cfg>(sm, ps.stage, &tA, &tAlo, &tB, &tBlo, a_mn0, b_mn0,
                              kb * Cfg::BLOCK_K + t.group * p.a_group_k, kb * Cfg::BLOCK_K + t.group * p.b_group_k, leader);
           ps.template advance<Cfg::STAGES>();
@@ -288,16 +325,16 @@
       }
     }
     __syncwarp();
-  } else if (warp == 1) {
+  } else if (warp == 1 && rank == 0) {
     const bool leader = elect_one();
     PipeState ps;
     int as = 0;
     uint32_t aphase = 0;
     int res_nblk = -1;
     uint32_t bphase = 0;
-    for (long long s = blockIdx.x; s < supers; s += gridDim.x) {
+    for (long long s = blockIdx.x / CTAS; s < supers; s += gridDim.x / CTAS) {
       for (int g = 0; g < g_loop; ++g) {
-        TileCoord t = gemm_decode(p, s, g, Cfg::BLOCK_K);
+        TileCoord t = gemm_decode(p, s, g, Cfg::BLOCK_K, CTAS, rank);
         if (Cfg::RES_KB > 0 && t.n_blk != res_nblk) {
           mbar_wait(sm.bfull, bphase);
           bphase ^= 1;
@@ -305,21 +342,21 @@
         }
         int n_rem = p.N - t.n_blk * Cfg::BLOCK_N;
         int n_eff = min(Cfg::BLOCK_N, (n_rem + 15) & ~15);
-        uint32_t idesc = make_idesc(Cfg::FMT, BLOCK_M, (uint32_t)n_eff, Cfg::A_MN ? 1u : 0u, Cfg::B_MN ? 1u : 0u);
+        uint32_t idesc = make_idesc(Cfg::FMT, Cfg::UMMA_M, (uint32_t)n_eff, Cfg::A_MN ? 1u : 0u, Cfg::B_MN ? 1u : 0u);
         const int chain = Cfg::PROMOTE_KB > 0 ? Cfg::PROMOTE_KB : (t.kb1 - t.kb0);
         for (int kc = t.kb0; kc < t.kb1; kc += chain) {
           int kce = min(t.kb1, kc + chain);
-          mbar_wait(&sm.tempty[as], aphase ^ 1);
+          pipe_wait<Cfg>(&sm.tempty[as], aphase ^ 1);
           tc_fence_after();
           for (int kb = kc; kb < kce; ++kb) {
-            mbar_wait(&sm.full[ps.stage], ps.phase);
+            pipe_wait<Cfg>(&sm.full[ps.stage], ps.phase);
             tc_fence_after();
             int kvalid = min(Cfg::BLOCK_K, p.K - kb * Cfg::BLOCK_K);
             issue_stage_rt<Cfg>(sm, ps.stage, tmem_base + as * Cfg::BLOCK_N, kvalid, kb == kc, idesc, kb - t.kb0, leader);
-            if (leader) mma_commit(&sm.empty[ps.stage]);
+            if (leader) mma_commit<Cfg::PAIR>(&sm.empty[ps.stage]);
             ps.template advance<Cfg::STAGES>();
           }
-          if (leader) mma_commit(&sm.tfull[as]);
+          if (leader) mma_commit<Cfg::PAIR>(&sm.tfull[as]);
           __syncwarp();
           as ^= 1;
           if (as == 0) aphase ^= 1;
@@ -341,17 +378,17 @@
       const int e = (p.exp_a ? __ldg(p.exp_a) : 0) + (p.exp_b ? __ldg(p.exp_b) : 0);
       acc_scale = exp2f((float)-e) * (p.post_scale != 0.f ? p.post_scale : 1.0f);
     }
-    for (long long s = blockIdx.x; s < supers; s += gridDim.x) {
-      TileCoord t = gemm_decode(p, s, 0, Cfg::BLOCK_K);
+    for (long long s = blockIdx.x / CTAS; s < supers; s += gridDim.x / CTAS) {
+      TileCoord t = gemm_decode(p, s, 0, Cfg::BLOCK_K, CTAS, rank);
       const int row = t.m_blk * BLOCK_M + quarter * 32 + lane;
       const int col0 = t.n_blk * Cfg::BLOCK_N + group_c * COLS;
       epi.tile_begin(p, t, row, col0);
-      if (s + gridDim.x < supers) {
-        const TileCoord t2 = gemm_decode(p, s + gridDim.x, 0, Cfg::BLOCK_K);
+      if (s + gridDim.x / CTAS < supers) {
+        const TileCoord t2 = gemm_decode(p, s + gridDim.x / CTAS, 0, Cfg::BLOCK_K, CTAS, rank);
         epi.tile_prefetch(p, t2, t2.m_blk * BLOCK_M + quarter * 32 + lane, t2.n_blk * Cfg::BLOCK_N + group_c * COLS);
       }
       if constexpr (Cfg::PROMOTE_KB == 0 && !Epi::kAccumulate) {
-        mbar_wait(&sm.tfull[as], aphase);
+        pipe_wait<Cfg>(&sm.tfull[as], aphase);
         tc_fence_after();
 #pragma unroll
         for (int i = 0; i < NCH; ++i) {
@@ -369,7 +406,7 @@
         }
         tc_fence_before();
         __syncwarp();
-        if (lane == 0) mbar_arrive(&sm.tempty[as]);
+        if (lane == 0) tmem_release<Cfg>(&sm.tempty[as]);
         as ^= 1;
         if (as == 0) aphase ^= 1;
       } else {
@@ -379,11 +416,11 @@
 #pragma unroll
           for (int j = 0; j < 32; ++j) accr[i][j] = 0.f;
         for (int g = 0; g < g_loop; ++g) {
-          t = gemm_decode(p, s, g, Cfg::BLOCK_K);
+          t = gemm_decode(p, s, g, Cfg::BLOCK_K, CTAS, rank);
           const float scale = epi.group_scale(p, t, row);
           const int chain = Cfg::PROMOTE_KB > 0 ? Cfg::PROMOTE_KB : (t.kb1 - t.kb0);
           for (int kc = t.kb0; kc < t.kb1; kc += chain) {
-            mbar_wait(&sm.tfull[as], aphase);
+            pipe_wait<Cfg>(&sm.tfull[as], aphase);
             tc_fence_after();
 #pragma unroll
             for (int i = 0; i < NCH; ++i) {
@@ -405,7 +442,7 @@
             }
             tc_fence_before();
             __syncwarp();
-            if (lane == 0) mbar_arrive(&sm.tempty[as]);
+            if (lane == 0) tmem_release<Cfg>(&sm.tempty[as]);
             as ^= 1;
             if (as == 0) aphase ^= 1;
           }
@@ -443,7 +480,7 @@
   constexpr bool bf16 = Cfg::ELEM == 2;
   int rc;
   uint32_t a_box_rows = Cfg::A_MN ? Cfg::BLOCK_K : BLOCK_M;
-  uint32_t b_box_rows = Cfg::B_MN ? Cfg::BLOCK_K : Cfg::BLOCK_N;
+  uint32_t b_box_rows = Cfg::B_MN ? Cfg::BLOCK_K : Cfg::B_ROWS;
   const bool a32 = Cfg::A_MN && Cfg::MN_ATOM32, b32 = Cfg::B_MN && Cfg::MN_ATOM32;
   if ((rc = make_tmap_2d(tA, A.main, Cfg::ELEM, bf16, A.rows, A.cols, A.pitch, Cfg::CHUNK, a_box_rows, a32))) return rc;
   if ((rc = make_tmap_2d(tB, B.main, Cfg::ELEM, bf16, B.rows, B.cols, B.pitch, Cfg::CHUNK, b_box_rows, b32))) return rc;
@@ -481,12 +518,32 @@
     if (!pp.exp_a) pp.exp_a = A.exp;
     if (!pp.exp_b) pp.exp_b = B.exp;
   }
-  const int sms = sm_count();
-  long long supers = (long long)p.m_tiles * p.n_tiles * p.splits * (p.groups_inner ? 1 : p.groups);
-  int grid = (int)(supers < sms ? supers : sms);
-  if (grid_override > 0 && grid_override < grid) grid = grid_override;
+  int slots = sm_count();
+  if (Cfg::PAIR) {
+    static int clusters[64] = {};
+    if (!clusters[dev]) {
+      cudaLaunchConfig_t cfg = {};
+      cfg.gridDim = dim3(2 * slots);
+      cfg.blockDim = dim3(Cfg::THREADS);
+      cfg.dynamicSmemBytes = Cfg::SMEM_BYTES;
+      cudaLaunchAttribute attr[1];
+      attr[0].id = cudaLaunchAttributeClusterDimension;
+      attr[0].val.clusterDim.x = 2; attr[0].val.clusterDim.y = 1; attr[0].val.clusterDim.z = 1;
+      cfg.attrs = attr;
+      cfg.numAttrs = 1;
+      int n = 0;
+      if ((rc = check_cuda(cudaOccupancyMaxActiveClusters(&n, umma_gemm_kernel<Cfg, Epi>, &cfg)))) return rc;
+      if (n < 1) return COPER_ERR_UNSUPPORTED;
+      clusters[dev] = n;
+    }
+    slots = clusters[dev];
+  }
+  const long long supers = gemm_supers(p, Cfg::CTAS);
+  int grid = (int)(supers < slots ? supers : slots);
+  if (grid_override > 0 && grid_override < grid * Cfg::CTAS) grid = grid_override / Cfg::CTAS;
   if (grid < 1) return COPER_ERR_INVALID_ARG;
-  launch_pdl(umma_gemm_kernel<Cfg, Epi>, grid, Cfg::THREADS, Cfg::SMEM_BYTES, st, tA, tAlo, tB, tBlo, pp, epi);
+  launch_pdl_cluster(umma_gemm_kernel<Cfg, Epi>, Cfg::CTAS, grid * Cfg::CTAS, Cfg::THREADS, Cfg::SMEM_BYTES, st, tA, tAlo,
+                     tB, tBlo, pp, epi);
   return check_launch();
 }
 
```

After: 1.021 million, median of 6. +2.1%, better.
